# KMS-TEAM/vi_slam

Hardware: AMD Instinct MI355X
Metric: frames/sec ORB extract+match (higher is better)
Workload: dtype u8; 1 GPU; kitti00_mono_1241x376_n1000; nfeatures=1000, nlevels=8, contexts_in_flight=4, distinct_frames=32, match=SearchForInitialization(prev frame) window 100

## Files before the change

include/vslam_fe.h:

```cpp
#ifndef VSLAM_FE_H
#define VSLAM_FE_H

#include <stddef.h>
#include <stdint.h>

#ifdef __cplusplus
extern "C" {
#endif

#define VSLAM_OK 0
#define VSLAM_ERR_INVALID (-1)
#define VSLAM_ERR_NO_DEVICE (-2)
#define VSLAM_ERR_HIP (-3)
#define VSLAM_ERR_CAPACITY (-4)
#define VSLAM_ERR_UNSUPPORTED (-5)
#define VSLAM_ERR_COMM (-6)

#define VSLAM_MAX_LEVELS 16
#define VSLAM_MAX_BATCH 64

#define VSLAM_IMGS_HOST 0
#define VSLAM_IMGS_DEVICE 1
#define VSLAM_IMGS_PINNED 2
#define VSLAM_IMGS_STAGED 3

#define VSLAM_FLAG_ATAN_FMA 1u
#define VSLAM_FLAG_HOST_OCTREE 2u

typedef struct vslam_kp {
    float x, y, size, angle, response;
    int32_t octave, class_id;
} vslam_kp;

typedef struct vslam_tuning {
    int32_t pyramid_per_level;
    int32_t pyr_rows;
    int32_t pyr_threads;
    int32_t blur_rows;
    int32_t fast_threads;
    int32_t fast_pitch;
    int32_t fast_lds_pad;
    int32_t octree_walk_kernel;
    int32_t oct_fine_depth;
    int32_t oct_lds_budget_kb;
    int32_t oct_regkeys;
    int32_t oct_max_iter;
    int32_t oct_debug;
    int32_t graphs;
    int32_t h2d_route;
    int32_t d2h_route;
    int32_t copy_wgs;
    int32_t pull_depth;
    int32_t init_topm;
    int32_t init_match_host;
    int32_t sbp_topm;
    int32_t sbp_sequential;
    int32_t si_queries_per_block;
    int32_t fg_threads;
    int32_t wait_spin;
    int32_t numa;
    int32_t host_prof;
    int32_t stream_priority;
    int32_t stage_split_event;
    int32_t oct_threads;
    int32_t fast_kernel;
    int32_t fast_band_cells;
    int32_t wave_prio;
    int32_t oct_precount;
    int32_t desc_kpw;
    int32_t reserved[1];
} vslam_tuning;
void vslam_tuning_init(vslam_tuning* t);

typedef struct vslam_fe_params {
    int32_t width, height;
    int32_t nfeatures;
    float scale_factor;
    int32_t nlevels;
    int32_t ini_th_fast;
    int32_t min_th_fast;
    int32_t device;
    int32_t max_batch;
    uint32_t flags;
    int32_t gauss_taps[7];
    const vslam_tuning* tuning;
} vslam_fe_params;

typedef struct vslam_fe vslam_fe;


int vslam_fe_create(const vslam_fe_params* params, vslam_fe** out);
int vslam_fe_set_tuning(vslam_fe* fe, const vslam_tuning* t);
void vslam_fe_destroy(vslam_fe* fe);
const char* vslam_last_error(void);

int vslam_fe_tables(const vslam_fe* fe, float* scale, float* inv_scale, float* sigma2, float* inv_sigma2,
                    int32_t* features_per_level);

int vslam_fe_extract(vslam_fe* fe, const uint8_t* img, size_t pitch, int lap0, int lap1, vslam_kp* kps,
                     uint8_t* desc, int cap, int* n, int* mono_index);

int vslam_fe_extract_batch(vslam_fe* fe, int nimg, const uint8_t* const* imgs, size_t pitch,
                           int imgs_on_device, int lap0, int lap1, vslam_kp* const* kps,
                           uint8_t* const* desc, int cap, int* n, int* mono_index);

int vslam_fe_stage_images_async(vslam_fe* fe, int nimg, const uint8_t* const* imgs, size_t pitch, int imgs_where);

int vslam_fe_extract_batch_async(vslam_fe* fe, int nimg, const uint8_t* const* imgs, size_t pitch,
                                 int imgs_on_device, int lap0, int lap1, int want_host);
int vslam_fe_extract_wait(vslam_fe* fe, vslam_kp* const* kps, uint8_t* const* desc, int cap, int* n,
                          int* mono_index);

int vslam_fe_level_size(const vslam_fe* fe, int level, int* w, int* h);

int vslam_fe_capacity(const vslam_fe* fe);
int vslam_fe_level_copy(vslam_fe* fe, int slot, int level, int blurred, uint8_t* dst, size_t dst_pitch);

int vslam_fe_candidates(vslam_fe* fe, int slot, int level, vslam_kp* out, int cap);

int vslam_fe_slot_buffers(vslam_fe* fe, int slot, const vslam_kp** dev_kps, const uint8_t** dev_desc,
                          int* n);

int vslam_fe_slot_host_views(vslam_fe* fe, int slot, const vslam_kp** host_kps, const uint8_t** host_desc);

int vslam_fe_wait_for(vslam_fe* waiter, vslam_fe* signal);
int vslam_fe_event_record(vslam_fe* fe, int idx);
int vslam_fe_event_wait(vslam_fe* waiter, vslam_fe* signal, int idx);

int vslam_fe_set_fast_gate(vslam_fe* fe, vslam_fe* signal);

void* vslam_fe_stream(vslam_fe* fe);

int vslam_fe_pack_slots(vslam_fe* fe, int nslots, void* dev_dst, size_t slot_bytes);
int vslam_fe_pack_slot_range(vslam_fe* fe, int first, int nslots, void* dev_dst, size_t slot_bytes);
int vslam_fe_pack_slot_range_async(vslam_fe* fe, int first, int nslots, void* dev_dst, size_t slot_bytes);

#define VSLAM_COMM_ID_BYTES 128
typedef struct vslam_comm vslam_comm;
int vslam_comm_unique_id(uint8_t id[VSLAM_COMM_ID_BYTES]);
int vslam_comm_create(int device, int rank, int world, const uint8_t id[VSLAM_COMM_ID_BYTES], vslam_comm** out);
void vslam_comm_destroy(vslam_comm* comm);
int vslam_comm_rank(const vslam_comm* comm);
int vslam_comm_world(const vslam_comm* comm);
int vslam_exchange_ring(vslam_fe* fe, vslam_comm* comm, const void* dev_send, void* dev_recv, size_t bytes);
int vslam_exchange_allgather(vslam_fe* fe, vslam_comm* comm, const void* dev_send, void* dev_recv_all,
                             size_t bytes_per_rank);

int vslam_host_alloc(size_t bytes, void** out);
void vslam_host_free(void* p);

int vslam_fe_set_profiling(vslam_fe* fe, int on);
int vslam_fe_get_profile(vslam_fe* fe, double stage_ms[5], long* batches, long* images);
// ... 147 lines not shown

int vslam_distinctive_descriptors(vslam_fe* fe, const uint8_t* desc_host, const int32_t* offsets, int nsets,
                                  int32_t* best);

typedef struct vslam_voc vslam_voc;
int vslam_voc_create(int device, int depth_levels, int weighting, int norm, int n_nodes, const int32_t* child_start,
                     const int32_t* child_count, const int32_t* child_ids, int n_child_ids, const uint8_t* node_desc,
                     const double* node_weight, const int32_t* node_word_id, vslam_voc** out);
void vslam_voc_destroy(vslam_voc* voc);
typedef struct vslam_voc_file vslam_voc_file;
int vslam_voc_file_open(const char* path, vslam_voc_file** out);
void vslam_voc_file_close(vslam_voc_file* f);
int vslam_voc_file_info(const vslam_voc_file* f, int* branching, int* depth_levels, int* scoring, int* weighting,
                        int* norm, int* n_nodes, int* n_words, int* n_child_ids, int* format);
int vslam_voc_file_arrays(const vslam_voc_file* f, const int32_t** child_start, const int32_t** child_count,
                          const int32_t** child_ids, const uint8_t** node_desc, const double** node_weight,
                          const int32_t** node_word_id);
const char* vslam_voc_file_last_error(void);
int vslam_voc_load(int device, const char* path, vslam_voc** out);
long vslam_dbg_qlz_decode(const uint8_t* packet, size_t n, uint8_t* dst, size_t cap, size_t* used);
int vslam_voc_info(const vslam_voc* voc, int* depth_levels, int* weighting, int* norm, int* n_nodes);
int vslam_bow_transform(vslam_fe* fe, const vslam_voc* voc, const uint8_t* dev_desc, int n, int levelsup,
                        int32_t* word_id, double* weight, int32_t* node_id);
int vslam_bow_transform_slots_async(vslam_fe* fe, const vslam_voc* voc, int first_slot, int nslots, int levelsup);
int vslam_bow_transform_slots_wait(vslam_fe* fe, const int* n, int32_t* const* word_id, double* const* weight,
                                   int32_t* const* node_id);
int vslam_bow_assemble(int weighting, int norm, const int32_t* word_id, const double* weight, const int32_t* node_id,
                       int n, int32_t* bow_ids, double* bow_vals, int* n_bow, int32_t* fv_nodes, int32_t* fv_off,
                       int32_t* fv_feat, int* n_fv);

int vslam_search_by_bow(vslam_fe* fe, const vslam_kp* kf_kps_host, const uint8_t* dev_kf_desc,
                        const uint8_t* kf_flags_host, int n_kf, const int32_t* kf_fv_nodes, const int32_t* kf_fv_off,
                        const int32_t* kf_fv_feat, int n_kf_nodes, const vslam_kp* f_kps_host,
                        const uint8_t* dev_f_desc, int n_f, const int32_t* f_fv_nodes, const int32_t* f_fv_off,
                        const int32_t* f_fv_feat, int n_f_nodes, float nnratio, int check_orientation,
                        int32_t* match_f, int* nmatches);

int vslam_search_by_bow_keyframes(vslam_fe* fe, const vslam_kp* kps1_host, const uint8_t* dev_desc1,
                                  const uint8_t* flags1_host, int n1, const int32_t* fv1_nodes, const int32_t* fv1_off,
                                  const int32_t* fv1_feat, int n1_nodes, const vslam_kp* kps2_host,
                                  const uint8_t* dev_desc2, const uint8_t* flags2_host, int n2,
                                  const int32_t* fv2_nodes, const int32_t* fv2_off, const int32_t* fv2_feat,
                                  int n2_nodes, float nnratio, int check_orientation, int32_t* match12, int* nmatches);

typedef struct vslam_tri_params {
    float F12[9];
    float ep_x, ep_y;
    int32_t only_stereo, coarse, check_orientation;
} vslam_tri_params;
int vslam_search_for_triangulation(vslam_fe* fe, const vslam_tri_params* p, const vslam_kp* kps1_host,
                                   const uint8_t* dev_desc1, const uint8_t* has_mp1_host, const float* u_right1_host,
                                   int n1, const int32_t* fv1_nodes, const int32_t* fv1_off, const int32_t* fv1_feat,
                                   int n1_nodes, const vslam_kp* kps2_host, const uint8_t* dev_desc2,
                                   const uint8_t* has_mp2_host, const float* u_right2_host, int n2,
                                   const int32_t* fv2_nodes, const int32_t* fv2_off, const int32_t* fv2_feat,
                                   int n2_nodes, int32_t* match12, int* nmatches);

typedef struct vslam_fuse_point {
    float pos[3];
    float normal[3];
    float min_distance;
    float max_distance;
    int32_t valid;
} vslam_fuse_point;
typedef struct vslam_fuse_params {
    float Rcw[9], tcw[3], Ow[3];
    float fx, fy, cx, cy, bf, th;
    float log_scale_factor;
    int32_t img_w, img_h;
    int32_t sim3;
    int32_t gemm_float;
    float Rb[9], tb[3];
} vslam_fuse_params;
int vslam_fuse_search(vslam_fe* fe, const vslam_fuse_params* p, const vslam_fuse_point* points_host,
                      const uint8_t* mp_desc_host, int n_points, const vslam_kp* dev_kf_kps,
                      const uint8_t* dev_kf_desc, int n_kf, const float* kf_u_right_host, int32_t* best_idx,
                      int32_t* best_dist);

int vslam_dbg_sincos(vslam_fe* fe, const float* x, int n, float* sin_out, float* cos_out);
int vslam_dbg_fast_atan2(vslam_fe* fe, const float* y, const float* x, int n, int fma, float* deg);
int vslam_dbg_logf(vslam_fe* fe, const float* x, int n, float* y);
int vslam_fe_octree_stats(const vslam_fe* fe, unsigned long long* problems, unsigned long long* split_below_grid,
                          uint32_t* last_level_masks);
int vslam_fe_delivery_stats(const vslam_fe* fe, unsigned long long* transfers, unsigned long long* bytes);
int vslam_dbg_octree_stamps(vslam_fe* fe, unsigned long long* out64);
int vslam_dbg_search_init_fallbacks(vslam_fe* fe, int* count);
int vslam_dbg_search_init_replay_stats(vslam_fe* fe, int* rounds, int* queries, int* pairs);

#ifdef __cplusplus
}
#endif
#endif
```

vi_slam_amd/__init__.py:

```python
import ctypes as C
import os

import numpy as np

_HERE = os.path.dirname(os.path.abspath(__file__))
LIB_PATH = os.environ.get("VSLAM_FE_LIB") or os.path.join(_HERE, "libvslam_fe.so")
HOST_LIB_PATH = os.path.join(_HERE, "libvslam_host.so")

VSLAM_OK = 0
ERR_INVALID, ERR_NO_DEVICE, ERR_HIP, ERR_CAPACITY, ERR_UNSUPPORTED, ERR_COMM = -1, -2, -3, -4, -5, -6
IMGS_HOST, IMGS_DEVICE, IMGS_PINNED, IMGS_STAGED = 0, 1, 2, 3
COMM_ID_BYTES = 128
FLAG_ATAN_FMA = 1
FLAG_HOST_OCTREE = 2
MAX_BATCH = 64

KP_DTYPE = np.dtype([("x", "<f4"), ("y", "<f4"), ("size", "<f4"), ("angle", "<f4"),
                     ("response", "<f4"), ("octave", "<i4"), ("class_id", "<i4")])

ABI_SYMBOLS = [
    "vslam_fe_create", "vslam_fe_destroy", "vslam_last_error", "vslam_fe_tables", "vslam_fe_extract",
    "vslam_fe_extract_batch", "vslam_fe_level_size", "vslam_fe_level_copy", "vslam_fe_candidates",
    "vslam_fe_slot_buffers", "vslam_fe_slot_host_views", "vslam_fe_capacity", "vslam_fe_stream", "vslam_hamming_top2", "vslam_hamming_matrix",
    "vslam_stereo_match", "vslam_stereo_match_batch", "vslam_search_for_initialization",
    "vslam_dbg_sincos", "vslam_dbg_fast_atan2", "vslam_fe_pack_slots", "vslam_fe_set_profiling",
    "vslam_fe_get_profile", "vslam_fe_extract_batch_async", "vslam_fe_extract_wait",
    "vslam_search_for_initialization_batch", "vslam_frame_stereo_batch_async", "vslam_frame_stereo_wait",
    "vslam_fe_pack_slot_range", "vslam_dbg_octree_stamps", "vslam_dbg_search_init_fallbacks", "vslam_search_init_dev_async",
    "vslam_search_init_dev_wait", "vslam_fe_slot_count_ptr", "vslam_fe_pack_slot_range_async", "vslam_fe_wait_for", "vslam_fe_event_record",
    "vslam_fe_event_wait", "vslam_projection_direction", "vslam_search_by_projection_frame",
    "vslam_search_by_projection_dev_async", "vslam_search_by_projection_dev_wait", "vslam_stereo_points_dev_async",
    "vslam_stereo_points_buffers", "vslam_search_by_projection_mappoints", "vslam_distinctive_descriptors", "vslam_voc_create", "vslam_voc_destroy",
    "vslam_voc_info", "vslam_bow_transform", "vslam_bow_transform_slots_async", "vslam_bow_transform_slots_wait",
    "vslam_bow_assemble", "vslam_search_by_bow", "vslam_search_by_bow_keyframes",
    "vslam_search_for_triangulation", "vslam_fuse_search", "vslam_dbg_logf", "vslam_search_by_projection_keyframe",
    "vslam_search_by_projection_sim3",
    "vslam_comm_unique_id", "vslam_comm_create", "vslam_comm_destroy", "vslam_comm_rank", "vslam_comm_world",
    "vslam_exchange_ring", "vslam_exchange_allgather", "vslam_host_alloc", "vslam_host_free",
    "vslam_fe_stage_images_async", "vslam_fe_octree_stats", "vslam_fe_delivery_stats", "vslam_dbg_search_init_replay_stats", "vslam_tuning_init", "vslam_fe_set_tuning", "vslam_stereo_fisheye_candidates", "vslam_hamming_top2_batch", "vslam_hamming_top2_batch_dev_async", "vslam_fe_set_fast_gate",
    "vslam_voc_load", "vslam_voc_file_open", "vslam_voc_file_close", "vslam_voc_file_info", "vslam_voc_file_arrays",
    "vslam_voc_file_last_error", "vslam_dbg_qlz_decode",
    "vslam_fe_set_camera", "vslam_fe_slot_ukps", "vslam_fe_ukps_copy", "vslam_undistort_points", "vslam_fe_image_bounds",
    "vslam_fe_set_grid_bounds", "vslam_fe_get_grid_bounds",
    "vslam_search_for_initialization_ex", "vslam_search_for_initialization_batch_ex", "vslam_search_init_dev_async_ex",
]


MP_TRACK_DTYPE = np.dtype([("proj_x", "<f4"), ("proj_y", "<f4"), ("proj_xr", "<f4"), ("view_cos", "<f4"),
                           ("level", "<i4"), ("flags", "<u4")])


FUSE_POINT_DTYPE = np.dtype([("pos", "<f4", 3), ("normal", "<f4", 3), ("min_distance", "<f4"),
                             ("max_distance", "<f4"), ("valid", "<i4")])


class _TriParams(C.Structure):
    _fields_ = [("F12", C.c_float * 9), ("ep_x", C.c_float), ("ep_y", C.c_float), ("only_stereo", C.c_int32),
                ("coarse", C.c_int32), ("check_orientation", C.c_int32)]


class _FuseParams(C.Structure):
    _fields_ = [("Rcw", C.c_float * 9), ("tcw", C.c_float * 3), ("Ow", C.c_float * 3), ("fx", C.c_float),
                ("fy", C.c_float), ("cx", C.c_float), ("cy", C.c_float), ("bf", C.c_float), ("th", C.c_float),
                ("log_scale_factor", C.c_float), ("img_w", C.c_int32), ("img_h", C.c_int32), ("sim3", C.c_int32),
                ("gemm_float", C.c_int32), ("Rb", C.c_float * 9), ("tb", C.c_float * 3)]


class _ProjParams(C.Structure):
    _fields_ = [("Tcw", C.c_float * 12), ("fx", C.c_float), ("fy", C.c_float), ("cx", C.c_float), ("cy", C.c_float),
                ("mbf", C.c_float), ("th", C.c_float), ("forward", C.c_int32), ("backward", C.c_int32),
                ("check_orientation", C.c_int32), ("img_w", C.c_int32), ("img_h", C.c_int32),
                ("gemm_float", C.c_int32)]


class _SbpJob(C.Structure):
    _fields_ = [("p", _ProjParams)] + [(n, C.c_void_p) for n in (
        "dev_last_kps", "dev_n_last", "dev_last_flags", "dev_last_x3dw", "dev_mp_desc", "dev_cur_kps", "dev_cur_desc",
        "dev_n_cur", "dev_cur_u_right", "dev_cur_occupied")]


class VslamError(RuntimeError):
    def __init__(self, code, msg):
        super().__init__("vslam error %d: %s" % (code, msg))
        self.code = code


TUNING_FIELDS = ["pyramid_per_level", "pyr_rows", "pyr_threads", "blur_rows", "fast_threads", "fast_pitch", "fast_lds_pad",
                 "octree_walk_kernel", "oct_fine_depth", "oct_lds_budget_kb", "oct_regkeys", "oct_max_iter",
                 "oct_debug", "graphs", "h2d_route", "d2h_route", "copy_wgs", "pull_depth",
                 "init_topm", "init_match_host", "sbp_topm", "sbp_sequential", "si_queries_per_block", "fg_threads",
                 "wait_spin", "numa", "host_prof", "stream_priority", "stage_split_event",
                 "oct_threads", "fast_kernel", "fast_band_cells", "wave_prio", "oct_precount", "desc_kpw"]


class _Tuning(C.Structure):
    _fields_ = [(f, C.c_int32) for f in TUNING_FIELDS] + [("reserved", C.c_int32 * 1)]


def make_tuning(**kw):
    t = _Tuning()
    lib().vslam_tuning_init(C.byref(t))
    for k, v in kw.items():
        if k not in TUNING_FIELDS:
            raise KeyError("unknown tuning field %r" % k)
        setattr(t, k, int(v))
    return t


class _Params(C.Structure):
    _fields_ = [("width", C.c_int32), ("height", C.c_int32), ("nfeatures", C.c_int32),
                ("scale_factor", C.c_float), ("nlevels", C.c_int32), ("ini_th_fast", C.c_int32),
                ("min_th_fast", C.c_int32), ("device", C.c_int32), ("max_batch", C.c_int32),
                ("flags", C.c_uint32), ("gauss_taps", C.c_int32 * 7), ("tuning", C.POINTER(_Tuning))]


class _InitJob(C.Structure):
    _fields_ = [("dev_kps1", C.c_void_p), ("dev_desc1", C.c_void_p), ("dev_n1", C.c_void_p),
                ("dev_kps2", C.c_void_p), ("dev_desc2", C.c_void_p), ("dev_n2", C.c_void_p),
                ("dev_prev_matched", C.c_void_p)]


class _Camera(C.Structure):
    _fields_ = [("fx", C.c_float), ("fy", C.c_float), ("cx", C.c_float), ("cy", C.c_float), ("dist", C.c_float * 5),
                ("ndist", C.c_int32)]


class _Bounds(C.Structure):
    _fields_ = [("min_x", C.c_float), ("max_x", C.c_float), ("min_y", C.c_float), ("max_y", C.c_float)]


def _bounds(b):
    return _Bounds(*[float(v) for v in b])


def bind_voc_file(L):
    vp = C.c_void_p
    L.vslam_voc_file_open.argtypes = [C.c_char_p, vp]
    L.vslam_voc_file_close.argtypes = [vp]
    L.vslam_voc_file_close.restype = None
    L.vslam_voc_file_info.argtypes = [vp] + [vp] * 9
    L.vslam_voc_file_arrays.argtypes = [vp] + [vp] * 6
    L.vslam_voc_file_last_error.restype = C.c_char_p
    L.vslam_dbg_qlz_decode.argtypes = [C.c_char_p, C.c_size_t, vp, C.c_size_t, vp]
    L.vslam_dbg_qlz_decode.restype = C.c_long
    return L


def qlz_decode(packet, library=None, cap=None):
    L = library if library is not None else lib()
    packet = bytes(packet)
    n = len(packet)
    if cap is None:
        cap = 16 + 128 * n
    dst = C.create_string_buffer(max(cap, 1))
    used = C.c_size_t(0)
    got = L.vslam_dbg_qlz_decode(packet, n, dst, cap, C.byref(used))
    if got < 0:
        raise ValueError("damaged QuickLZ packet")
    return dst.raw[:got], used.value


_lib = None


def lib():
    global _lib
    if _lib is None:
        if not os.path.exists(LIB_PATH):
            raise ImportError("%s is missing: run `python -c 'import __graft_entry__ as g; g.build()'` "
                              "(make -C vi_slam_amd/csrc); there is no CPU fallback" % LIB_PATH)
        try:
            import torch
        except Exception:
            pass
        L = C.CDLL(LIB_PATH)
# ... 354 lines not shown
        if len(d) not in (4, 5):
            raise VslamError(ERR_INVALID, "dist must hold 4 or 5 coefficients")
        cam = _Camera(fx, fy, cx, cy, (C.c_float * 5)(*(d + [0.0] * (5 - len(d)))), len(d))
        _check(lib().vslam_fe_set_camera(self._h, C.byref(cam)))

    def slot_ukps_ptr(self, slot=0):
        k = C.c_void_p()
        _check(lib().vslam_fe_slot_ukps(self._h, slot, C.byref(k)))
        return k.value

    def ukeypoints(self, slot=0):
        out = np.zeros(self.cap, KP_DTYPE)
        n = C.c_int()
        _check(lib().vslam_fe_ukps_copy(self._h, slot, _p(out), self.cap, C.byref(n)))
        return out[:n.value].copy()

    def image_bounds(self):
        b = np.zeros(4, np.float32)
        _check(lib().vslam_fe_image_bounds(self._h, _p(b)))
        return b

    def set_grid_bounds(self, bounds):
        if bounds is None:
            _check(lib().vslam_fe_set_grid_bounds(self._h, None))
            return
        b = _bounds(bounds)
        _check(lib().vslam_fe_set_grid_bounds(self._h, C.byref(b)))

    def grid_bounds(self):
        b, s = _Bounds(), C.c_int()
        _check(lib().vslam_fe_get_grid_bounds(self._h, C.byref(b), C.byref(s)))
        return np.array([b.min_x, b.max_x, b.min_y, b.max_y], np.float32), bool(s.value)

    def wait_for(self, other):
        _check(lib().vslam_fe_wait_for(self._h, other._h))

    def event_record(self, idx):
        _check(lib().vslam_fe_event_record(self._h, idx))

    def set_fast_gate(self, other):
        L = lib()
        L.vslam_fe_set_fast_gate.argtypes = [C.c_void_p, C.c_void_p]
        _check(L.vslam_fe_set_fast_gate(self._h, other._h if other is not None else None))

    def event_wait(self, other, idx):
        _check(lib().vslam_fe_event_wait(self._h, other._h, idx))

    def stream(self):
        return lib().vslam_fe_stream(self._h)

    @property
    def slot_bytes(self):
        return (16 + self.cap * 60 + 255) & ~255

    def pack_slots(self, nslots, dev_dst, slot_bytes=None, first=0, sync=True):
        fn = lib().vslam_fe_pack_slot_range if sync else lib().vslam_fe_pack_slot_range_async
        _check(fn(self._h, first, nslots, dev_dst, slot_bytes or self.slot_bytes))

    def stereo_points_async(self, Twc, cam, observations=True, gemm_float=False):
        T = np.ascontiguousarray(np.asarray(Twc, np.float32).reshape(len(Twc), -1)[:, :12])
        _check(lib().vslam_stereo_points_dev_async(self._h, len(Twc), _p(T), C.c_float(cam[0]), C.c_float(cam[1]),
                                                   C.c_float(cam[2]), C.c_float(cam[3]), int(observations),
                                                   int(gemm_float)))

    def stereo_points_buffers(self, pair, with_stereo=True):
        x, f, u, d = C.c_void_p(), C.c_void_p(), C.c_void_p(), C.c_void_p()
        _check(lib().vslam_stereo_points_buffers(self._h, pair, C.byref(x), C.byref(f),
                                                 C.byref(u) if with_stereo else None,
                                                 C.byref(d) if with_stereo else None))
        return x.value, f.value, u.value, d.value

    def set_tuning(self, **kw):
        t = make_tuning(**kw)
        lib().vslam_fe_set_tuning.argtypes = [C.c_void_p, C.c_void_p]
        _check(lib().vslam_fe_set_tuning(self._h, C.byref(t)))

    def octree_stats(self):
        a, b = C.c_ulonglong(), C.c_ulonglong()
        m = (C.c_uint32 * MAX_BATCH)()
        lib().vslam_fe_octree_stats.argtypes = [C.c_void_p, C.c_void_p, C.c_void_p, C.c_void_p]
        _check(lib().vslam_fe_octree_stats(self._h, C.byref(a), C.byref(b), m))
        return a.value, b.value, [int(v) for v in m]

    def delivery_stats(self):
        a, b = C.c_ulonglong(), C.c_ulonglong()
        lib().vslam_fe_delivery_stats.argtypes = [C.c_void_p, C.c_void_p, C.c_void_p]
        _check(lib().vslam_fe_delivery_stats(self._h, C.byref(a), C.byref(b)))
        return a.value, b.value

    def set_profiling(self, on=True):
        _check(lib().vslam_fe_set_profiling(self._h, int(on)))

    def get_profile(self):
        ms = (C.c_double * 5)()
        b, im = C.c_long(), C.c_long()
        _check(lib().vslam_fe_get_profile(self._h, ms, C.byref(b), C.byref(im)))
        return dict(pyramid_ms=ms[0], fast_ms=ms[1], blur_ms=ms[2], describe_ms=ms[3], octree_ms=ms[4],
                    batches=b.value, images=im.value)


class FMatcher:

    TH_HIGH, TH_LOW, HISTO_LENGTH = 100, 50, 30

    def __init__(self, extractor, nnratio=0.6, checkOri=True):
        self.fe = extractor
        self.mfNNratio = nnratio
        self.mbCheckOrientation = checkOri

    def hamming_top2(self, dev_q, nq, dev_t, nt):
        idx = np.zeros((max(nq, 1), 2), np.int32)
        dist = np.zeros((max(nq, 1), 2), np.int32)
        _check(lib().vslam_hamming_top2(self.fe._h, dev_q, nq, dev_t, nt, _p(idx), _p(dist)))
        return idx[:nq], dist[:nq]

    def hamming_top2_batch(self, problems):
        n = len(problems)
        idx = [np.zeros((max(p[1], 1), 2), np.int32) for p in problems]
        dist = [np.zeros((max(p[1], 1), 2), np.int32) for p in problems]
        vp, ip = C.c_void_p * n, C.c_int32 * n
        L = lib()
        L.vslam_hamming_top2_batch.argtypes = [C.c_void_p, C.c_int, C.c_void_p, C.c_void_p, C.c_void_p, C.c_void_p, C.c_void_p, C.c_void_p]
        _check(L.vslam_hamming_top2_batch(self.fe._h, n, vp(*[p[0] for p in problems]), ip(*[p[1] for p in problems]),
                                          vp(*[p[2] for p in problems]), ip(*[p[3] for p in problems]),
                                          vp(*[a.ctypes.data for a in idx]), vp(*[a.ctypes.data for a in dist])))
        return [(idx[i][:problems[i][1]], dist[i][:problems[i][1]]) for i in range(n)]

    def hamming_top2_batch_async(self, problems):
        n = len(problems)
        vp, ip = C.c_void_p * n, C.c_int32 * n
        L = lib()
        L.vslam_hamming_top2_batch_dev_async.argtypes = [C.c_void_p, C.c_int, C.c_void_p, C.c_void_p, C.c_void_p, C.c_void_p]
        _check(L.vslam_hamming_top2_batch_dev_async(self.fe._h, n, vp(*[p[0] for p in problems]), ip(*[p[1] for p in problems]),
                                                    vp(*[p[2] for p in problems]), ip(*[p[3] for p in problems])))

    def ComputeStereoFishEyeCandidates(self, dev_desc_left, n_left, mono_left, dev_desc_right, n_right, mono_right):
        l2r = np.zeros(max(n_left, 1), np.int32)
        d0 = np.zeros(max(n_left, 1), np.int32)
        d1 = np.zeros(max(n_left, 1), np.int32)
        nc = C.c_int()
        L = lib()
        L.vslam_stereo_fisheye_candidates.argtypes = [C.c_void_p, C.c_void_p, C.c_int, C.c_int, C.c_void_p, C.c_int, C.c_int,
                                                      C.c_void_p, C.c_void_p, C.c_void_p, C.c_void_p]
        _check(L.vslam_stereo_fisheye_candidates(self.fe._h, dev_desc_left, n_left, mono_left, dev_desc_right, n_right,
                                                 mono_right, _p(l2r), _p(d0), _p(d1), C.byref(nc)))
        return l2r[:n_left], d0[:n_left], d1[:n_left], nc.value

    def hamming_matrix(self, dev_q, nq, dev_t, nt):
        out = np.zeros((max(nq, 1), max(nt, 1)), np.uint8)
        _check(lib().vslam_hamming_matrix(self.fe._h, dev_q, nq, dev_t, nt, _p(out)))
        return out[:nq, :nt]

    def SearchForInitialization(self, kps1, dev_desc1, kps2, dev_desc2, vbPrevMatched, windowSize=10,
                                img_size=None, bounds=None):
        kps1 = np.ascontiguousarray(kps1, KP_DTYPE)
        kps2 = np.ascontiguousarray(kps2, KP_DTYPE)
        pm = np.ascontiguousarray(vbPrevMatched, np.float32).copy()
        m = np.full(max(len(kps1), 1), -1, np.int32)
        nm = C.c_int(0)
        if bounds is not None:
            _check(lib().vslam_search_for_initialization_ex(self.fe._h, _p(kps1), dev_desc1, len(kps1), _p(kps2),
                                                            dev_desc2, len(kps2), C.byref(_bounds(bounds)), _p(pm), _p(m),
                                                            windowSize, self.mfNNratio, int(self.mbCheckOrientation),
                                                            C.byref(nm)))
            return nm.value, m[:len(kps1)], pm
        w, h = img_size or (self.fe.width, self.fe.height)
# ... 484 lines not shown
```

vi_slam_amd/csrc/vslam_ctx.h:

```cpp
#ifndef VSLAM_CTX_H
#define VSLAM_CTX_H
#include <hip/hip_runtime.h>

#include <algorithm>
#include <atomic>
#include <cmath>
#include <condition_variable>
#include <cstdio>
#include <cstring>
#include <functional>
#include <mutex>
#include <string>
#include <thread>
#include <vector>

#include "../../include/vslam_orb_pattern.h"
#include "vslam_host.h"
#include "vslam_pool.h"
#include "vslam_kernels.h"
#include "vslam_tuning.h"

std::string& vslam_err();
#define g_err (vslam_err())

#define HIPCHK(call)                                                                             \
    do {                                                                                         \
        hipError_t e_ = (call);                                                                  \
        if (e_ != hipSuccess) {                                                                  \
            g_err = std::string(#call) + ": " + hipGetErrorString(e_);                           \
            return VSLAM_ERR_HIP;                                                                \
        }                                                                                        \
    } while (0)

enum { VSLAM_REGION_NONE = 0, VSLAM_REGION_INIT = 1, VSLAM_REGION_STEREO = 2 };
struct vslam_fe {
    vslam_fe_params p;
    vslam_tuning tune;
    vslam::ExtractorTables tab;
    PyramidGeom geom;
    size_t slot_stride = 0;
    int B = 1, cap = 0;

    hipStream_t stream = nullptr;
    hipEvent_t ev_cand = nullptr;
    hipEvent_t ev_x = nullptr;
    hipEvent_t ev_user[4] = {};
    int desc_kpw_hint = -1;
    hipEvent_t ev_fast = nullptr;
    vslam_fe* fast_gate = nullptr;
    bool fast_gated_by_someone = false;
    std::vector<vslam_fe*> gate_waiters;

    uint8_t* d_pyr = nullptr;
    uint8_t* d_blur = nullptr;
    uint16_t* d_xtab[VSLAM_MAX_LEVELS] = {};
    int16_t* d_xa[VSLAM_MAX_LEVELS] = {};
    uint16_t* d_ytab[VSLAM_MAX_LEVELS] = {};
    int16_t* d_yb[VSLAM_MAX_LEVELS] = {};
    uint16_t* d_qbase[VSLAM_MAX_LEVELS] = {};
    ResizeQuad* d_quads[VSLAM_MAX_LEVELS] = {};
    struct PyrGroupCtx {
        PyrGroupDev dev;
        size_t lds_bytes;
        PyrTileDev* d_tiles;
    };
    std::vector<PyrGroupCtx> pyr_groups;
    std::vector<vslam::HostCell> cells;
    int level_cell_first[VSLAM_MAX_LEVELS + 1] = {};
    CellDesc* d_cells = nullptr;
    int tile_pitch = 0, tile_rows = 0, max_px = 0;
    BandDesc* d_bands = nullptr;
    uint8_t* d_band_classes = nullptr;
    int nbands = 0, band_max_wh = 0, band_max_iw = 0;
    uint8_t* d_cand = nullptr;
    uint8_t* h_cand = nullptr;
    size_t cand_stride = 0;
    int cand_cap = 0;
    int32_t taps[7];
    uint32_t* d_blur_tasks = nullptr;
    int n_blur_tasks = 0;
    int oct_threads = 1024;
    int blur_rows = 32;
    SelKp* d_sel = nullptr;
    SelKp* h_sel = nullptr;
    uint8_t* d_res = nullptr;
    uint8_t* h_res = nullptr;
    size_t res_bytes = 0, res_counts_bytes = 0, res_feat_bytes = 0, res_init_bytes = 0;
    bool init_in_block = false;
    unsigned long long n_deliveries = 0, n_delivery_bytes = 0, graph_deliveries = 0, graph_delivery_bytes = 0;
    bool deliver_deferred = false;
    vslam_kp* d_kps = nullptr;
    uint8_t* d_desc = nullptr;
    vslam_kp* h_kps = nullptr;
    uint8_t* h_desc = nullptr;
    int8_t* d_pattern = nullptr;
    BatchSrc src;
    int n_out[VSLAM_MAX_BATCH] = {};
    int mono_out[VSLAM_MAX_BATCH] = {};
    unsigned long long oct_problems = 0, oct_deep = 0;
    uint32_t oct_last_mask[VSLAM_MAX_BATCH] = {};
    int32_t pack_hdr[VSLAM_MAX_BATCH][4] = {};
    std::vector<std::vector<vslam::Cand>> sel_level;
    std::vector<std::vector<vslam::Cand>> cand_level;
    uint8_t* h_top2 = nullptr;
    size_t h_top2_bytes = 0;
    uint32_t* d_part = nullptr;
    size_t part_bytes = 0;
    int32_t* d_idx2 = nullptr;
    int32_t* d_dist2 = nullptr;
    size_t top2_cap = 0;
    uint8_t* d_dmat = nullptr;
    size_t dmat_bytes = 0;
    uint8_t* d_tmp_desc[2] = {nullptr, nullptr};
    size_t tmp_desc_bytes[2] = {0, 0};
    uint8_t* d_init = nullptr;
    size_t init_bytes = 0;
    uint8_t* h_init = nullptr;
    size_t h_init_bytes = 0;
    int init_pairs = 0;
    bool init_lds_set = false;
    bool has_cam = false;
    UdCam ud;
    vslam_kp* d_ukps = nullptr;
    bool has_grid_bounds = false;
    SiBounds grid_bounds = {0.0f, 0.0f, 0.0f, 0.0f};
    uint8_t* d_init_scratch = nullptr;
    size_t init_scratch_bytes = 0;
    int* d_init_fb = nullptr;
    uint8_t* d_proj = nullptr;
    size_t proj_bytes = 0;
    uint8_t* h_proj = nullptr;
    size_t h_proj_bytes = 0;
    bool proj_lds_set = false, dist_lds_set = false;
    uint8_t* d_bow = nullptr;
    size_t bow_bytes = 0;
    uint8_t* h_bow = nullptr;
    size_t h_bow_bytes = 0;
    int bow_jobs = 0;
    bool use_graph = true;
    hipGraphExec_t graph_exec = nullptr;
    long long graph_key = 0;
    size_t graph_pitch = 0;
    const uint8_t* graph_imgs[VSLAM_MAX_BATCH] = {};
    int graph_lap0 = 0, graph_lap1 = 0;
    uint8_t* h_img = nullptr;
    size_t h_img_pitch = 0;
    uint8_t* d_stage = nullptr;
    size_t d_stage_bytes = 0;
    uint8_t* d_sbp = nullptr;
// ... 81 lines not shown
```

vi_slam_amd/csrc/vslam_fe.hip:

```cpp
#if defined(__SSE2__)
#include <emmintrin.h>
#endif
#include "vslam_ctx.h"

#include <algorithm>
#include <chrono>
#include <mutex>
#include <cstdio>
#include <cstdlib>

void vslam_host_prof_report();

std::string& vslam_err() {
    static thread_local std::string e;
    return e;
}
extern "C" const char* vslam_last_error(void) { return vslam_err().c_str(); }

static std::mutex g_gate_mu;

static void gate_unlink(vslam_fe* fe) {
    if (fe->fast_gate) {
        auto& w = fe->fast_gate->gate_waiters;
        w.erase(std::remove(w.begin(), w.end(), fe), w.end());
// ... 74 lines not shown
        if (fe->ev_prof[i]) hipEventDestroy(fe->ev_prof[i]);
    if (fe->stream) hipStreamDestroy(fe->stream);
    delete fe;
}

extern "C" void vslam_fe_destroy(vslam_fe* fe) {
    if (fe) hipSetDevice(fe->p.device);
    vslam_host_prof_report();
    free_ctx(fe);
}

#define UPLOAD(dst, ptr, bytes)                                                                  \
    do {                                                                                         \
        const size_t n_ = (bytes);                                                               \
        HIPCHK(hipMalloc((void**)&(dst), n_ ? n_ : 4));                                          \
        if (n_) HIPCHK(hipMemcpy((dst), (ptr), n_, hipMemcpyHostToDevice));                      \
    } while (0)


static int create_geometry(vslam_fe* fe) {
    const vslam_fe_params& p = fe->p;
    vslam::build_tables(p.nfeatures, p.scale_factor, p.nlevels, fe->tab);
    fe->B = p.max_batch;
    static const int32_t def_taps[7] = {18, 34, 48, 56, 48, 34, 18};
    bool zero = true;
    for (int i = 0; i < 7; i++) zero = zero && p.gauss_taps[i] == 0;
    for (int i = 0; i < 7; i++) fe->taps[i] = zero ? def_taps[i] : p.gauss_taps[i];

    memset(&fe->geom, 0, sizeof(fe->geom));
    fe->geom.nlevels = p.nlevels;
    int lws[VSLAM_MAX_LEVELS], lhs[VSLAM_MAX_LEVELS];
    size_t off = 0;
    for (int l = 0; l < p.nlevels; l++) {
        int lw, lh;
        vslam::level_size(fe->tab, p.width, p.height, l, &lw, &lh);
        LevelGeom& g = fe->geom.lv[l];
        g.w = lws[l] = lw;
        g.h = lhs[l] = lh;
        g.pitch = (lw + 127) & ~127;
        g.off = (uint32_t)off;
        g.scale = fe->tab.scale[l];
        off += (size_t)g.pitch * lh;
        off = (off + 255) & ~(size_t)255;
        if (lw < 40 || lh < 40 || lw > 4095 + 32 || lh > 4095 + 32) {
            g_err = "image too small/large for this level count";
            return VSLAM_ERR_UNSUPPORTED;
        }
        if ((int)std::round((float)(lw - 32) / (float)(lh - 32)) < 1) {
            g_err = "portrait aspect ratio: the reference's DistributeOctTree has nIni == 0 (undefined)";
            return VSLAM_ERR_UNSUPPORTED;
        }
    }
    fe->slot_stride = off;
    fe->cap = vslam::keypoint_capacity(fe->tab.quota.data(), lws, lhs, p.nlevels, p.nfeatures);
    HIPCHK(hipMalloc((void**)&fe->d_pyr, fe->slot_stride * fe->B));
    HIPCHK(hipMalloc((void**)&fe->d_blur, fe->slot_stride * fe->B));
    HIPCHK(hipMemset(fe->d_pyr, 0, fe->slot_stride * fe->B));
    HIPCHK(hipMemset(fe->d_blur, 0, fe->slot_stride * fe->B));
    return VSLAM_OK;
}

static int create_pyramid(vslam_fe* fe) {
    const vslam_fe_params& p = fe->p;
    std::vector<vslam::PyrLevelTables> pyr_tabs(p.nlevels);
    for (int l = 1; l < p.nlevels; l++) {
        vslam::ResizeTables& r = pyr_tabs[l].r;
        const LevelGeom &s = fe->geom.lv[l - 1], &d = fe->geom.lv[l];
        pyr_tabs[l].sw = s.w; pyr_tabs[l].sh = s.h; pyr_tabs[l].dw = d.w; pyr_tabs[l].dh = d.h;
        vslam::build_resize_tables(s.w, s.h, d.w, d.h, r);
        UPLOAD(fe->d_xtab[l], r.xtab.data(), r.xtab.size() * 2);
        UPLOAD(fe->d_xa[l], r.xa.data(), r.xa.size() * 2);
        UPLOAD(fe->d_ytab[l], r.ytab.data(), r.ytab.size() * 2);
        UPLOAD(fe->d_yb[l], r.yb.data(), r.yb.size() * 2);
        std::vector<uint16_t>& qbase = pyr_tabs[l].qbase;
        std::vector<uint32_t>& quads = pyr_tabs[l].quads;
        if (vslam::build_resize_quads(r, s.w, d.w, qbase, quads)) {
            UPLOAD(fe->d_qbase[l], qbase.data(), qbase.size() * 2);
            UPLOAD(fe->d_quads[l], quads.data(), quads.size() * 4);
        } else {
            qbase.clear();
            quads.clear();
        }
    }
    bool fused = fe->tune.pyramid_per_level != 1 && p.nlevels > 1;
    for (int l = 1; l < p.nlevels && fused; l++) fused = fe->d_quads[l] != nullptr;
    static_assert(sizeof(PyrTileDev) == sizeof(vslam::PyrTileLevel), "planner and kernel share the tile record");
    const int pyr_rows = fe->tune.pyr_rows >= 0 ? fe->tune.pyr_rows
                         : fe->B <= 2 ? 16 : (size_t)p.width * p.height > 1000000 ? 40 : 48;
#ifndef VSLAM_PYR_LDS_KB
#define VSLAM_PYR_LDS_KB 64
#endif
    for (int l0 = 0; fused && l0 + 1 < p.nlevels;) {
        const int nl = std::min(l0 == 0 ? 3 : VSLAM_PYR_GROUP_LEVELS, p.nlevels - 1 - l0);
        std::vector<const vslam::PyrLevelTables*> gt;
        for (int j = 1; j <= nl; j++) gt.push_back(&pyr_tabs[l0 + j]);
        vslam::PyrGroupPlan plan;
        if (!vslam::build_pyramid_group(gt, l0, VSLAM_PYR_LDS_KB * 1024, plan, pyr_rows)) {
            fused = false;
            break;
        }
        vslam_fe::PyrGroupCtx g;
        memset(&g.dev, 0, sizeof(g.dev));
        g.dev.l0 = l0;
        g.dev.nl = nl;
        g.dev.ntiles = plan.ntx * plan.nty;
        g.dev.readable_w0 = p.width;
        g.lds_bytes = plan.lds_bytes;
        g.d_tiles = nullptr;
        UPLOAD(g.d_tiles, plan.tiles.data(), plan.tiles.size() * sizeof(PyrTileDev));
        g.dev.tiles = g.d_tiles;
        for (int j = 0; j <= nl; j++) g.dev.lg[j] = fe->geom.lv[l0 + j];
        for (int j = 1; j <= nl; j++) {
            g.dev.qbase[j - 1] = fe->d_qbase[l0 + j];
            g.dev.quads[j - 1] = fe->d_quads[l0 + j];
            g.dev.ytab[j - 1] = fe->d_ytab[l0 + j];
            g.dev.yb[j - 1] = fe->d_yb[l0 + j];
        }
        fe->pyr_groups.push_back(g);
        l0 += nl;
    }
    if (!fused) {
        for (auto& g : fe->pyr_groups) hipFree(g.d_tiles);
        fe->pyr_groups.clear();
    }
    return VSLAM_OK;
}

static int create_fast(vslam_fe* fe) {
    const vslam_fe_params& p = fe->p;
    for (int l = 0; l < p.nlevels; l++) {
        fe->level_cell_first[l] = (int)fe->cells.size();
        vslam::build_cells(l, fe->geom.lv[l].w, fe->geom.lv[l].h, fe->cells);
    }
    fe->level_cell_first[p.nlevels] = (int)fe->cells.size();
    if (fe->cells.empty()) {
        g_err = "image too small: no 30-px FAST cell fits on any pyramid level";
        return VSLAM_ERR_UNSUPPORTED;
    }
    int maxw = 8, maxh = 8;
    size_t cand_total = 0;
    std::vector<CellDesc> dc(fe->cells.size());
    for (size_t i = 0; i < fe->cells.size(); i++) {
        const vslam::HostCell& c = fe->cells[i];
        dc[i].level = c.level; dc[i].x0 = c.x0; dc[i].y0 = c.y0; dc[i].x1 = c.x1; dc[i].y1 = c.y1; dc[i].pad = 0;
        dc[i].base = (uint32_t)cand_total;
        cand_total += (size_t)((c.x1 - c.x0 - 6 + 1) / 2) * (size_t)((c.y1 - c.y0 - 6 + 1) / 2);
        maxw = std::max(maxw, c.x1 - c.x0);
        maxh = std::max(maxh, c.y1 - c.y0);
    }
    fe->tile_pitch = (maxw + 3) & ~3;
    fe->tile_rows = maxh;
    fe->max_px = (maxw - 6) * (maxh - 6);
    if (fe->max_px > 8192) {
        g_err = "FAST cell larger than 8192 px";
        return VSLAM_ERR_UNSUPPORTED;
    }
    if (maxw > 66 || maxh > 134 || fe->geom.lv[p.nlevels - 1].w < 8) {
        g_err = "FAST cell window larger than 66 x 134 px";
        return VSLAM_ERR_UNSUPPORTED;
    }
    UPLOAD(fe->d_cells, dc.data(), dc.size() * sizeof(CellDesc));
    std::vector<vslam::HostBand> hb;
    vslam::build_bands(fe->cells, std::min(4, std::max(1, tune_or(fe->tune.fast_band_cells, 4))), 128, hb);
    vslam::BandTables bt;
    vslam::pack_bands(hb, p.nlevels, bt);
    static_assert(sizeof(BandDesc) == sizeof(vslam::BandWords), "packer and kernel share the band record");
    if (bt.ok && vk_fast_bands_check(bt.max_wh, bt.max_iw, bt.max_cells) == 0) {
        UPLOAD(fe->d_band_classes, bt.classes.data(), bt.classes.size());
        UPLOAD(fe->d_bands, bt.bands.data(), bt.bands.size() * sizeof(BandDesc));
        fe->nbands = (int)bt.bands.size();
        fe->band_max_wh = bt.max_wh;
        fe->band_max_iw = bt.max_iw;
    }
    fe->cand_cap = (int)std::max<size_t>(cand_total, 16);
    fe->cand_stride = (8 + fe->cells.size() * sizeof(CellOut) + (size_t)fe->cand_cap * 4 + 255) & ~(size_t)255;
    HIPCHK(hipMalloc((void**)&fe->d_cand, fe->cand_stride * fe->B));
    HIPCHK((hipError_t)vslam_pinned_alloc((void**)&fe->h_cand, fe->cand_stride * fe->B));
    return VSLAM_OK;
}

static int create_blur(vslam_fe* fe) {
    UPLOAD(fe->d_pattern, VSLAM_ORB_PATTERN, 1024);
    vk_upload_disc(fe->tab.umax);
    if (fe->tune.blur_rows >= 0) fe->blur_rows = std::min(512, std::max(8, (int)fe->tune.blur_rows));
    else if (fe->B <= 2) fe->blur_rows = 8;
    std::vector<uint32_t> tasks;
    for (int l = 0; l < fe->p.nlevels; l++) {
        const int br = fe->blur_rows;
        const int ns = std::max(1, (fe->geom.lv[l].w + 247) / 248), nc = (fe->geom.lv[l].h + br - 1) / br;
        for (int c = 0; c < nc; c++)
            for (int s = 0; s < ns; s++) tasks.push_back(((uint32_t)l << 24) | ((uint32_t)c << 12) | (uint32_t)s);
    }
    fe->n_blur_tasks = (int)tasks.size();
    UPLOAD(fe->d_blur_tasks, tasks.data(), tasks.size() * 4);
    return VSLAM_OK;
}

static int create_result_block(vslam_fe* fe) {
    const size_t nk = (size_t)fe->B * fe->cap;
    HIPCHK(hipMalloc((void**)&fe->d_sel, nk * sizeof(SelKp)));
    HIPCHK((hipError_t)vslam_pinned_alloc((void**)&fe->h_sel, nk * sizeof(SelKp)));
    fe->res_counts_bytes = (((size_t)(fe->B * 4 + 4) * 4) + 255) & ~(size_t)255;
    fe->res_feat_bytes = fe->res_counts_bytes + nk * sizeof(vslam_kp) + nk * 32;
    fe->res_init_bytes = (nk * 12 + (size_t)fe->B * 16 + 255) & ~(size_t)255;
    fe->res_bytes = fe->res_feat_bytes + fe->res_init_bytes;
    HIPCHK(hipMalloc((void**)&fe->d_res, fe->res_bytes));
    HIPCHK((hipError_t)vslam_pinned_alloc((void**)&fe->h_res, fe->res_bytes));
    HIPCHK(hipMemset(fe->d_res, 0, fe->res_bytes));
    memset(fe->h_res, 0, fe->res_bytes);
    fe->d_counts = (int32_t*)fe->d_res;
    fe->h_counts = (int32_t*)fe->h_res;
    fe->d_kps = (vslam_kp*)(fe->d_res + fe->res_counts_bytes);
    fe->h_kps = (vslam_kp*)(fe->h_res + fe->res_counts_bytes);
    fe->d_desc = fe->d_res + fe->res_counts_bytes + nk * sizeof(vslam_kp);
    fe->h_desc = fe->h_res + fe->res_counts_bytes + nk * sizeof(vslam_kp);
    fe->d_init = fe->d_res + fe->res_feat_bytes;
    fe->h_init = fe->h_res + fe->res_feat_bytes;
    fe->init_bytes = fe->h_init_bytes = fe->res_init_bytes;
    fe->init_in_block = true;
    return VSLAM_OK;
}

static int create_quadtree(vslam_fe* fe) {
    const vslam_fe_params& p = fe->p;
    int lws[VSLAM_MAX_LEVELS], lhs[VSLAM_MAX_LEVELS];
    for (int l = 0; l < p.nlevels; l++) {
        lws[l] = fe->geom.lv[l].w;
        lhs[l] = fe->geom.lv[l].h;
    }
    const size_t budget = (size_t)std::min(150, std::max(16, tune_or(fe->tune.oct_lds_budget_kb, 128))) * 1024;
    vslam::OctPlan plan;
    vslam::plan_octree(fe->tab.quota.data(), lws, lhs, fe->level_cell_first, p.nlevels, fe->tune.oct_fine_depth, budget,
                       vk_octree_lds_bytes, plan);
    OctParams& O = fe->oct;
    memset(&O, 0, sizeof(O));
    for (int l = 0; l < p.nlevels; l++) {
        O.N[l] = plan.N[l]; O.H[l] = plan.H[l]; O.nIni[l] = plan.nIni[l]; O.hX[l] = plan.hX[l];
        O.selOff[l] = plan.selOff[l]; O.fineD[l] = plan.fineD[l]; O.lutOff[l] = plan.lutOff[l]; O.lutW[l] = plan.lutW[l];
    }
    for (int l = 0; l <= p.nlevels; l++) O.cellFirst[l] = fe->level_cell_first[l];
    O.selStride = plan.selStride;
    O.maxNodes = plan.maxNodes;
    O.fineLdsOff = plan.fineLdsOff;
    O.fineLdsBytes = plan.fineLdsBytes;
    O.ptsCap = fe->cand_cap;
    if (fe->tune.oct_debug == 1) {
        HIPCHK(hipMalloc(&O.dbg, 64 * 8));
        HIPCHK(hipMemset(O.dbg, 0, 64 * 8));
    }
    O.maxIter = tune_or(fe->tune.oct_max_iter, 64);
    const bool on_device = fe->dev_octree = plan.fits && !(p.flags & VSLAM_FLAG_HOST_OCTREE);
    fe->oct_threads = fe->tune.oct_threads == 256 || fe->tune.oct_threads == 512 || fe->tune.oct_threads == 1024
                          ? fe->tune.oct_threads
                          : fe->B <= 2 ? 1024 : (size_t)p.width * p.height > 1000000 ? 512 : 256;
    if (!on_device) return VSLAM_OK;
    if (vk_octree_set_max_lds((size_t)O.fineLdsOff + (size_t)O.fineLdsBytes + 16) != 0) {
        g_err = "hipFuncSetAttribute(k_octree, max dynamic LDS) failed";
        return VSLAM_ERR_HIP;
    }
    const size_t np = (size_t)fe->B * fe->cand_cap;
    HIPCHK(hipMalloc((void**)&fe->d_pts[0], np * 4));
    HIPCHK(hipMalloc((void**)&fe->d_pts[1], np * 4));
    HIPCHK(hipMalloc((void**)&fe->d_sel_xyr, (size_t)fe->B * O.selStride * 4));
    HIPCHK(hipMalloc((void**)&fe->d_sel_cnt, (size_t)fe->B * VSLAM_MAX_LEVELS * 4));
    HIPCHK(hipMalloc((void**)&fe->d_oct_sorted, np * 8));
    HIPCHK(hipMalloc((void**)&fe->d_oct_redo, (size_t)fe->B * VSLAM_MAX_LEVELS * 4));
    HIPCHK(hipMemset(fe->d_oct_redo, 0, (size_t)fe->B * VSLAM_MAX_LEVELS * 4));
    UPLOAD(fe->d_oct_lut, plan.lut.data(), plan.lut.size() * 4);
    O.lut = fe->d_oct_lut;
    return VSLAM_OK;
}

static int create_stream_and_pool(vslam_fe* fe) {
    const int pr = tune_or(fe->tune.stream_priority, 0);
    int lo = 0, hi = 0;
    if (pr != 0 && hipDeviceGetStreamPriorityRange(&lo, &hi) == hipSuccess && lo != hi)
        HIPCHK(hipStreamCreateWithPriority(&fe->stream, hipStreamNonBlocking, pr == 1 ? lo : hi));
// ... 8 lines not shown
    nthreads = std::min(nthreads, fe->B * fe->p.nlevels - 1);
    fe->pool = new WorkerPool(std::max(nthreads, 0));
    return VSLAM_OK;
}

static int create_impl(vslam_fe* fe) {
    int ndev = 0;
    if (hipGetDeviceCount(&ndev) != hipSuccess || ndev <= 0 || fe->p.device >= ndev) {
        g_err = "no usable HIP device (this library has no CPU fallback)";
        return VSLAM_ERR_NO_DEVICE;
    }
    HIPCHK(hipSetDevice(fe->p.device));
    int (*const steps[])(vslam_fe*) = {create_geometry, create_pyramid, create_fast, create_blur, create_result_block,
                                       create_quadtree, create_stream_and_pool};
    for (auto step : steps) {
        const int rc = step(fe);
        if (rc != VSLAM_OK) return rc;
    }
    HIPCHK(hipDeviceSynchronize());
    return VSLAM_OK;
}

extern "C" int vslam_fe_create(const vslam_fe_params* p, vslam_fe** out) {
    if (!p || !out) return VSLAM_ERR_INVALID;
    *out = nullptr;
    if (p->width <= 0 || p->height <= 0 || p->nfeatures <= 0 || p->nlevels < 1 ||
        p->nlevels > VSLAM_MAX_LEVELS || p->scale_factor <= 1.0f || p->max_batch < 1 ||
        p->max_batch > VSLAM_MAX_BATCH || p->min_th_fast < 1 || p->ini_th_fast < p->min_th_fast ||
        p->ini_th_fast > 254 || p->nfeatures > 60000) {
        g_err = "invalid parameters";
        return VSLAM_ERR_INVALID;
    }
    vslam_fe* fe = new vslam_fe();
    fe->p = *p;
    fe->tune = vslam_resolve_tuning(p->tuning);
    fe->p.tuning = nullptr;
    int rc = create_impl(fe);
    if (rc != VSLAM_OK) {
        std::string keep = g_err;
        free_ctx(fe);
        g_err = keep;
        return rc;
    }
    *out = fe;
    return VSLAM_OK;
}

extern "C" int vslam_fe_set_tuning(vslam_fe* fe, const vslam_tuning* t) {
    if (!fe || !t) return VSLAM_ERR_INVALID;
    vslam_apply_tuning(fe->tune, t);
    fe->use_graph = fe->use_graph && fe->tune.graphs != 0;
    if (fe->graph_exec) {
        if (fe->stream) hipStreamSynchronize(fe->stream);
        hipGraphExecDestroy(fe->graph_exec);
        fe->graph_exec = nullptr;
        fe->graph_key = 0;
    }
    return VSLAM_OK;
}

extern "C" int vslam_fe_tables(const vslam_fe* fe, float* scale, float* inv_scale, float* sigma2,
                               float* inv_sigma2, int32_t* quota) {
    if (!fe) return VSLAM_ERR_INVALID;
    for (int i = 0; i < fe->p.nlevels; i++) {
        if (scale) scale[i] = fe->tab.scale[i];
        if (inv_scale) inv_scale[i] = fe->tab.inv_scale[i];
        if (sigma2) sigma2[i] = fe->tab.sigma2[i];
        if (inv_sigma2) inv_sigma2[i] = fe->tab.inv_sigma2[i];
        if (quota) quota[i] = fe->tab.quota[i];
    }
    return fe->p.nlevels;
}

extern "C" int vslam_fe_octree_stats(const vslam_fe* fe, unsigned long long* problems, unsigned long long* split_below_grid,
                                     uint32_t* last_level_masks) {
    if (!fe) return VSLAM_ERR_INVALID;
    if (problems) *problems = fe->oct_problems;
    if (split_below_grid) *split_below_grid = fe->oct_deep;
    if (last_level_masks)
        for (int s = 0; s < fe->B; s++) last_level_masks[s] = s < fe->last_nimg ? fe->oct_last_mask[s] : 0u;
    return VSLAM_OK;
}

extern "C" int vslam_fe_delivery_stats(const vslam_fe* fe, unsigned long long* transfers, unsigned long long* bytes) {
    if (!fe) return VSLAM_ERR_INVALID;
    if (transfers) *transfers = fe->n_deliveries;
    if (bytes) *bytes = fe->n_delivery_bytes;
    return VSLAM_OK;
}

extern "C" int vslam_dbg_octree_stamps(vslam_fe* fe, unsigned long long* out64) {
    if (!fe || !fe->oct.dbg) return VSLAM_ERR_INVALID;
    HIPCHK(hipMemcpy(out64, fe->oct.dbg, 64 * 8, hipMemcpyDeviceToHost));
    return VSLAM_OK;
}

extern "C" void* vslam_fe_stream(vslam_fe* fe) { return fe ? (void*)fe->stream : nullptr; }

extern "C" int vslam_fe_wait_for(vslam_fe* waiter, vslam_fe* signal) {
    if (!waiter || !signal || waiter->p.device != signal->p.device) return VSLAM_ERR_INVALID;
    if (waiter == signal) return VSLAM_OK;
    HIPCHK(hipSetDevice(waiter->p.device));
    if (!signal->ev_x) HIPCHK(hipEventCreateWithFlags(&signal->ev_x, hipEventDisableTiming));
    HIPCHK(hipEventRecord(signal->ev_x, signal->stream));
    HIPCHK(hipStreamWaitEvent(waiter->stream, signal->ev_x, 0));
    return VSLAM_OK;
}

extern "C" int vslam_fe_event_record(vslam_fe* fe, int idx) {
    if (!fe || idx < 0 || idx >= 4) return VSLAM_ERR_INVALID;
    HIPCHK(hipSetDevice(fe->p.device));
    if (!fe->ev_user[idx]) HIPCHK(hipEventCreateWithFlags(&fe->ev_user[idx], hipEventDisableTiming));
    HIPCHK(hipEventRecord(fe->ev_user[idx], fe->stream));
    return VSLAM_OK;
}

extern "C" int vslam_fe_event_wait(vslam_fe* waiter, vslam_fe* signal, int idx) {
    if (!waiter || !signal || idx < 0 || idx >= 4 || waiter->p.device != signal->p.device) return VSLAM_ERR_INVALID;
    if (!signal->ev_user[idx] || waiter == signal) return VSLAM_OK;
    HIPCHK(hipSetDevice(waiter->p.device));
    HIPCHK(hipStreamWaitEvent(waiter->stream, signal->ev_user[idx], 0));
    return VSLAM_OK;
}

extern "C" int vslam_fe_set_fast_gate(vslam_fe* fe, vslam_fe* signal) {
    if (!fe || (signal && (signal == fe || signal->p.device != fe->p.device))) return VSLAM_ERR_INVALID;
    std::lock_guard<std::mutex> lk(g_gate_mu);
    gate_unlink(fe);
    if (signal) {
        fe->fast_gate = signal;
        signal->gate_waiters.push_back(fe);
        HIPCHK(hipSetDevice(signal->p.device));
        if (!signal->ev_fast) HIPCHK(hipEventCreateWithFlags(&signal->ev_fast, hipEventDisableTiming));
        signal->fast_gated_by_someone = true;
        fe->use_graph = false;
        signal->use_graph = false;
    }
    return VSLAM_OK;
}

extern "C" int vslam_fe_set_profiling(vslam_fe* fe, int on) {
    if (!fe) return VSLAM_ERR_INVALID;
    HIPCHK(hipSetDevice(fe->p.device));
    if (on && !fe->ev_prof[0])
        for (int i = 0; i < 10; i++) HIPCHK(hipEventCreate(&fe->ev_prof[i]));
    fe->profiling = on != 0;
    for (int i = 0; i < 5; i++) fe->prof_ms[i] = 0;
    fe->prof_batches = fe->prof_images = 0;
    return VSLAM_OK;
}

extern "C" int vslam_fe_get_profile(vslam_fe* fe, double stage_ms[5], long* batches, long* images) {
    if (!fe || !stage_ms) return VSLAM_ERR_INVALID;
    for (int i = 0; i < 5; i++) stage_ms[i] = fe->prof_ms[i];
    if (batches) *batches = fe->prof_batches;
    if (images) *images = fe->prof_images;
    return VSLAM_OK;
}

static int pack_range(vslam_fe* fe, int first, int nslots, void* dev_dst, size_t slot_bytes, bool sync) {
    if (!fe || first < 0 || nslots < 0 || first + nslots > fe->B || !dev_dst ||
        slot_bytes < 16 + (size_t)fe->cap * 60 || (slot_bytes & 15) || ((uintptr_t)dev_dst & 15)) {
        g_err = "invalid arguments (slot_bytes and dev_dst must be 16-byte aligned)";
        return VSLAM_ERR_INVALID;
    }
    HIPCHK(hipSetDevice(fe->p.device));
// ... 128 lines not shown
    const bool use_sdma = h2d_uses_sdma(fe, nimg);
    BatchSrc hs;
    for (int s = 0; s < nimg; s++) {
        if (where == VSLAM_IMGS_PINNED && !imgs[s]) {
            g_err = "null image";
            return VSLAM_ERR_INVALID;
        }
        hs.l0[s] = where == VSLAM_IMGS_PINNED ? imgs[s] : fe->h_img + img_bytes * s;
        hs.pitch0[s] = where == VSLAM_IMGS_PINNED ? (uint32_t)pitch : (uint32_t)fe->h_img_pitch;
    }
    int from_host = 1;
    if (use_sdma) {
        const size_t spitch = hs.pitch0[0];
        const size_t one = (size_t)(p.height - 1) * spitch + p.width;
        const size_t stride = (one + 255) & ~(size_t)255;
        if (fe->d_stage_bytes < stride * fe->B + 256) {
            g_err = "internal: device staging buffer not allocated";
            return VSLAM_ERR_HIP;
        }
        hipStream_t cs = st;
        bool even = nimg > 1;
        const ptrdiff_t d = nimg > 1 ? hs.l0[1] - hs.l0[0] : 0;
        for (int s = 2; s < nimg && even; s++) even = hs.l0[s] - hs.l0[s - 1] == d;
        if (even && d > 0 && (size_t)d >= one && (size_t)d * (nimg - 1) + one <= fe->d_stage_bytes) {
            const int ek = fe->tune.stage_split_event;
            const int h1 = nimg / 2;
            if (ek >= 0 && ek < 4 && h1 >= 1 && !hip_stream_capturing(cs)) {
                HIPCHK(hipMemcpyAsync(fe->d_stage, hs.l0[0], (size_t)d * h1, hipMemcpyHostToDevice, cs));
                if (!fe->ev_user[ek]) HIPCHK(hipEventCreateWithFlags(&fe->ev_user[ek], hipEventDisableTiming));
                HIPCHK(hipEventRecord(fe->ev_user[ek], cs));
                HIPCHK(hipMemcpyAsync(fe->d_stage + (size_t)d * h1, hs.l0[0] + (size_t)d * h1, (size_t)d * (nimg - 1 - h1) + one,
                                      hipMemcpyHostToDevice, cs));
            } else
                HIPCHK(hipMemcpyAsync(fe->d_stage, hs.l0[0], (size_t)d * (nimg - 1) + one, hipMemcpyHostToDevice, cs));
            for (int s = 0; s < nimg; s++) hs.l0[s] = fe->d_stage + (size_t)d * s;
        } else {
            for (int s = 0; s < nimg; s++) {
                HIPCHK(hipMemcpyAsync(fe->d_stage + stride * s, hs.l0[s], one, hipMemcpyHostToDevice, cs));
                hs.l0[s] = fe->d_stage + stride * s;
            }
        }
        from_host = 0;
    }
    vk_pull_images(st, hs, fe->d_pyr, fe->slot_stride, fe->geom.lv[0].off, (int)lp, p.width, p.height, nimg, from_host, fe->tune);
    return VSLAM_OK;
}

static void src_at_slots(vslam_fe* fe, int nimg) {
    for (int s = 0; s < nimg; s++) {
        fe->src.l0[s] = fe->d_pyr + (size_t)s * fe->slot_stride + fe->geom.lv[0].off;
        fe->src.pitch0[s] = (uint32_t)fe->geom.lv[0].pitch;
    }
}

static int enqueue_front(vslam_fe* fe, int nimg, const uint8_t* const* imgs, size_t pitch, int on_device) {
    const vslam_fe_params& p = fe->p;
    const int L = p.nlevels;
    hipStream_t st = fe->stream;
    if (on_device == VSLAM_IMGS_DEVICE) {
        for (int s = 0; s < nimg; s++) {
            if (!imgs[s]) {
                g_err = "null image";
                return VSLAM_ERR_INVALID;
            }
            fe->src.l0[s] = imgs[s];
            fe->src.pitch0[s] = (uint32_t)pitch;
        }
    } else {
        if (on_device != VSLAM_IMGS_STAGED) {
            int rc = upload_host_rows(fe, nimg, imgs, pitch, on_device);
            if (rc) return rc;
        }
        src_at_slots(fe, nimg);
    }
    fe->last_nimg = nimg;
    fe->cand_on_host = false;
    int32_t* d_errw = fe->dev_octree ? fe->d_counts + (size_t)fe->B * 4 : nullptr;
    if (fe->pyr_groups.empty()) vk_reset_headers(st, fe->d_cand, fe->cand_stride, nimg, d_errw);
    const bool prof = fe->profiling;
    if (prof) HIPCHK(hipEventRecord(fe->ev_prof[0], st));
    bool first_group = true;
    for (const auto& g : fe->pyr_groups) {
        vk_pyramid_group(st, fe->d_pyr, fe->slot_stride, fe->src, g.dev, g.lds_bytes, nimg,
                         first_group ? fe->d_cand : nullptr, fe->cand_stride, first_group ? d_errw : nullptr);
        first_group = false;
    }
    for (int l = 1; l < L && fe->pyr_groups.empty(); l++) {
        if (fe->d_quads[l])
            vk_resize_level_v2(st, fe->d_pyr, fe->slot_stride, fe->src, fe->geom.lv[l - 1], fe->geom.lv[l], l - 1,
                               fe->d_qbase[l], fe->d_quads[l], fe->d_ytab[l], fe->d_yb[l], nimg);
        else
            vk_resize_level(st, fe->d_pyr, fe->slot_stride, fe->src, fe->geom.lv[l - 1], fe->geom.lv[l], l - 1,
                            fe->d_xtab[l], fe->d_xa[l], fe->d_ytab[l], fe->d_yb[l], nimg);
    }
    if (prof) HIPCHK(hipEventRecord(fe->ev_prof[1], st));
    if (fe->fast_gate && fe->fast_gate->ev_fast) HIPCHK(hipStreamWaitEvent(st, fe->fast_gate->ev_fast, 0));
    if (fe->nbands > 0 && tune_or(fe->tune.fast_kernel, fe->B <= 2 ? 3 : 4) != 3)
        vk_fast_bands(st, fe->d_pyr, fe->slot_stride, fe->src, fe->geom, fe->d_bands, fe->nbands, fe->d_band_classes, fe->d_cells,
                      (int)fe->cells.size(), fe->d_cand, fe->cand_stride, p.ini_th_fast, p.min_th_fast, fe->band_max_wh, fe->band_max_iw, nimg);
    else
        vk_fast_cells_v3(st, fe->d_pyr, fe->slot_stride, fe->src, fe->geom, fe->d_cells, (int)fe->cells.size(), fe->d_cand,
                         fe->cand_stride, p.ini_th_fast, p.min_th_fast, fe->tile_rows, fe->tile_pitch, fe->max_px, nimg);
    if (fe->fast_gated_by_someone && fe->ev_fast) HIPCHK(hipEventRecord(fe->ev_fast, st));
    if (prof) HIPCHK(hipEventRecord(fe->ev_prof[2], st));
    return VSLAM_OK;
}

static int fetch_candidates(vslam_fe* fe, int nimg) {
    const size_t hdr_bytes = 8 + fe->cells.size() * sizeof(CellOut);
    HIPCHK(hipMemcpy2DAsync(fe->h_cand, fe->cand_stride, fe->d_cand, fe->cand_stride, hdr_bytes + (size_t)fe->cand_cap * 4,
                            nimg, hipMemcpyDeviceToHost, fe->stream));
    HIPCHK(hipEventRecord(fe->ev_cand, fe->stream));
    return VSLAM_OK;
}

static int wait_candidates(vslam_fe* fe, int nimg) {
    HIPCHK(hipEventSynchronize(fe->ev_cand));
    for (int s = 0; s < nimg; s++) {
        const uint32_t* hdr = (const uint32_t*)(fe->h_cand + (size_t)s * fe->cand_stride);
        if (hdr[1]) {
            g_err = "FAST candidate buffer overflow";
            return VSLAM_ERR_CAPACITY;
        }
    }
    fe->cand_on_host = true;
    return VSLAM_OK;
}

static int enqueue_blur(vslam_fe* fe, int nimg) {
    if (fe->profiling) HIPCHK(hipEventRecord(fe->ev_prof[3], fe->stream));
    vk_blur7_v2(fe->stream, fe->d_pyr, fe->slot_stride, fe->src, fe->geom, fe->d_blur, fe->d_blur_tasks,
                fe->n_blur_tasks, fe->taps, fe->blur_rows, nimg);
    if (fe->profiling) HIPCHK(hipEventRecord(fe->ev_prof[4], fe->stream));
    return VSLAM_OK;
}

static int select_host(vslam_fe* fe, int nimg, int lap0, int lap1) {
    const int L = fe->p.nlevels;
    hipStream_t st = fe->stream;
    int rc = fetch_candidates(fe, nimg);
    if (rc == VSLAM_OK) rc = enqueue_blur(fe, nimg);
    if (rc) return rc;
    HIPCHK(hipGetLastError());
    if ((rc = wait_candidates(fe, nimg))) return rc;
    std::atomic<int> bad(0);
    fe->pool->parallel_for(nimg * L, [&](int task) {
        const int s = task / L, l = task % L;
        decode_candidates(fe, s, l);
        const std::vector<vslam::Cand>& cl = fe->cand_level[(size_t)s * L + l];
        const LevelGeom& g = fe->geom.lv[l];
        if (!vslam::distribute_octree(cl.data(), (int)cl.size(), g.w - 2 * VSLAM_FAST_BORDER,
                                      g.h - 2 * VSLAM_FAST_BORDER, fe->tab.quota[l],
                                      fe->sel_level[(size_t)s * L + l]))
            bad++;
    });
    if (bad.load()) {
        g_err = "DistributeOctTree: nIni == 0";
        return VSLAM_ERR_UNSUPPORTED;
    }
    for (int s = 0; s < nimg; s++) {
        int nk = 0;
        for (int l = 0; l < L; l++) nk += (int)fe->sel_level[(size_t)s * L + l].size();
        if (nk > fe->cap) {
            g_err = "internal keypoint capacity exceeded";
            return VSLAM_ERR_CAPACITY;
        }
        SelKp* sel = fe->h_sel + (size_t)s * fe->cap;
        int monoIndex = 0, stereoIndex = nk - 1;
        for (int l = 0; l < L; l++) {
            const float scale = fe->tab.scale[l];
            for (const vslam::Cand& c : fe->sel_level[(size_t)s * L + l]) {
                const int lx = c.x + VSLAM_FAST_BORDER, ly = c.y + VSLAM_FAST_BORDER;
                float px = (float)lx;
                if (l != 0) px = px * scale;
                SelKp k;
                k.x = (uint16_t)lx;
                k.y = (uint16_t)ly;
                k.level = (uint8_t)l;
                k.slot = (uint8_t)s;
                k.response = c.response;
                k.pad = 0;
                k.out = (px >= (float)lap0 && px <= (float)lap1) ? (uint32_t)stereoIndex-- : (uint32_t)monoIndex++;
                *sel++ = k;
            }
        }
        fe->h_counts[s * 4] = nk;
        fe->h_counts[s * 4 + 1] = monoIndex;
        fe->h_counts[s * 4 + 2] = 0;
    }
    fe->h_counts[fe->B * 4] = 0;
    HIPCHK(hipMemcpyAsync(fe->d_counts, fe->h_counts, (size_t)(fe->B * 4 + 4) * 4, hipMemcpyHostToDevice, st));
    HIPCHK(hipMemcpyAsync(fe->d_sel, fe->h_sel, (size_t)nimg * fe->cap * sizeof(SelKp), hipMemcpyHostToDevice, st));
    if (fe->profiling) {
        HIPCHK(hipEventRecord(fe->ev_prof[7], st));
        HIPCHK(hipEventRecord(fe->ev_prof[8], st));
    }
    return VSLAM_OK;
}

static int select_dev(vslam_fe* fe, int nimg, int lap0, int lap1) {
    hipStream_t st = fe->stream;
    int32_t* d_err = fe->d_counts + (size_t)fe->B * 4;
    const int rc = enqueue_blur(fe, nimg);
    if (rc) return rc;
    if (fe->profiling) HIPCHK(hipEventRecord(fe->ev_prof[7], st));
    vk_octree(st, fe->d_cand, fe->cand_stride, (int)fe->cells.size(), fe->oct, fe->d_pts[0], fe->d_pts[1],
              fe->d_oct_sorted, (size_t)fe->cand_cap, fe->d_sel_xyr, fe->d_sel_cnt, d_err, fe->p.nlevels, nimg,
              fe->d_oct_redo, fe->tune.oct_regkeys, fe->oct_threads);
    vk_assign_out(st, fe->oct, fe->geom, fe->d_sel_xyr, fe->d_sel_cnt, lap0, lap1, fe->d_sel, fe->d_counts, fe->cap,
                  d_err, nimg, fe->d_oct_redo);
    if (fe->profiling) HIPCHK(hipEventRecord(fe->ev_prof[8], st));
    return VSLAM_OK;
}

static int enqueue_back(vslam_fe* fe, int nimg, int lap0, int lap1) {
// ... 582 lines not shown
```

vi_slam_amd/csrc/vslam_host.cpp:

```cpp
#include "vslam_host.h"
#include "vslam_undistort.h"

#include <algorithm>
#include <climits>
#include <cmath>
#include <cstdlib>
#include <cstring>

namespace vslam {

static inline int cv_round(float v) { return (int)lrintf(v); }
static inline int cv_round(double v) { return (int)lrint(v); }
static inline int cv_floor(float v) {
    int i = (int)v;
    return i - (i > v);
}
static inline int cv_ceil(float v) {
    int i = (int)v;
    return i + (i < v);
}
static inline int16_t sat_short(float v) {
    int iv = cv_round(v);
    return (int16_t)std::min(std::max(iv, (int)SHRT_MIN), (int)SHRT_MAX);
}
// ... 32 lines not shown
    for (v = 0; v <= vmax; ++v) t.umax[v] = cv_round(sqrt(hp2 - v * v));
    for (v = HP, v0 = 0; v >= vmin; --v) {
        while (t.umax[v0] == t.umax[v0 + 1]) ++v0;
        t.umax[v] = v0;
        ++v0;
    }
    t.disc_u.clear();
    t.disc_v.clear();
    for (v = -HP; v <= HP; v++) {
        const int d = t.umax[std::abs(v)];
        for (int u = -d; u <= d; u++) {
            t.disc_u.push_back((int8_t)u);
            t.disc_v.push_back((int8_t)v);
        }
    }
}

void level_size(const ExtractorTables& t, int w, int h, int level, int* lw, int* lh) {
    const float scale = t.inv_scale[level];
    *lw = cv_round((float)w * scale);
    *lh = cv_round((float)h * scale);
}

void build_resize_tables(int sw, int sh, int dw, int dh, ResizeTables& r) {
    const int ONE = 2048;
    const double scale_x = 1. / ((double)dw / sw), scale_y = 1. / ((double)dh / sh);
    r.xtab.resize(2 * dw);
    r.xa.resize(2 * dw);
    r.ytab.resize(2 * dh);
    r.yb.resize(2 * dh);
    for (int dx = 0; dx < dw; dx++) {
        float fx = (float)((dx + 0.5) * scale_x - 0.5);
        int sx = cv_floor(fx);
        fx -= sx;
        if (sx < 0) { fx = 0; sx = 0; }
        if (sx >= sw - 1) { fx = 0; sx = sw - 1; }
        r.xtab[2 * dx] = (uint16_t)sx;
        r.xtab[2 * dx + 1] = (uint16_t)std::min(sx + 1, sw - 1);
        r.xa[2 * dx] = sat_short((1.f - fx) * ONE);
        r.xa[2 * dx + 1] = sat_short(fx * ONE);
    }
    auto clip = [](int x, int a, int b) { return x >= a ? (x < b ? x : b - 1) : a; };
    for (int dy = 0; dy < dh; dy++) {
        float fy = (float)((dy + 0.5) * scale_y - 0.5);
        int sy = cv_floor(fy);
        fy -= sy;
        r.ytab[2 * dy] = (uint16_t)clip(sy, 0, sh);
        r.ytab[2 * dy + 1] = (uint16_t)clip(sy + 1, 0, sh);
        r.yb[2 * dy] = sat_short((1.f - fy) * ONE);
        r.yb[2 * dy + 1] = sat_short(fy * ONE);
    }
}

bool build_resize_quads(const ResizeTables& r, int sw, int dw, std::vector<uint16_t>& qbase,
                        std::vector<uint32_t>& quads) {
    if (sw < 8) return false;
    const int nq = (dw + 3) / 4;
    qbase.assign(nq, 0);
    quads.assign((size_t)nq * 8, 0);
    for (int q = 0; q < nq; q++) {
        int lo = 1 << 30, hi = -1;
        for (int j = 0; j < 4; j++) {
            const int dx = std::min(4 * q + j, dw - 1);
            lo = std::min(lo, (int)r.xtab[2 * dx]);
            hi = std::max(hi, (int)r.xtab[2 * dx + 1]);
        }
        const int base = std::min(lo, sw - 8);
        if (hi - base > 7) return false;
        qbase[q] = (uint16_t)base;
        for (int j = 0; j < 4; j++) {
            const int dx = std::min(4 * q + j, dw - 1);
            const uint32_t o0 = r.xtab[2 * dx] - base, o1 = r.xtab[2 * dx + 1] - base;
            quads[(size_t)q * 8 + j] = o0 | (0x0cu << 8) | (o1 << 16) | (0x0cu << 24);
            quads[(size_t)q * 8 + 4 + j] = (uint32_t)(uint16_t)r.xa[2 * dx] | ((uint32_t)(uint16_t)r.xa[2 * dx + 1] << 16);
        }
    }
    return true;
}


static inline int div_floor4(int x) { return x >> 2; }

static bool plan_with(const std::vector<const PyrLevelTables*>& tabs, int l0, int ntx, int nty, size_t max_lds,
                      PyrGroupPlan& plan) {
    const int nl = (int)tabs.size();
    plan.l0 = l0;
    plan.nl = nl;
    plan.ntx = ntx;
    plan.nty = nty;
    plan.tiles.assign((size_t)ntx * nty * (nl + 1), PyrTileLevel{});
    size_t lds_max = 0;
    for (int ty = 0; ty < nty; ty++)
        for (int tx = 0; tx < ntx; tx++) {
            PyrTileLevel* T = &plan.tiles[((size_t)ty * ntx + tx) * (nl + 1)];
            int cq0[VSLAM_MAX_LEVELS + 1], cq1[VSLAM_MAX_LEVELS + 1], cr0[VSLAM_MAX_LEVELS + 1], cr1[VSLAM_MAX_LEVELS + 1];
            int nq0 = -1, nq1 = -1, nr0 = -1, nr1 = -1;
            for (int j = nl; j >= 0; j--) {
                int oq0 = 0, oq1 = 0, or0 = 0, or1 = 0;
                if (j >= 1) {
                    const PyrLevelTables& t = *tabs[j - 1];
                    const int nq = (t.dw + 3) / 4;
                    oq0 = (int)((long long)tx * nq / ntx);
                    oq1 = (int)((long long)(tx + 1) * nq / ntx);
                    or0 = (int)((long long)ty * t.dh / nty);
                    or1 = (int)((long long)(ty + 1) * t.dh / nty);
                    T[j].sq0 = (int16_t)oq0; T[j].sq1 = (int16_t)oq1; T[j].sr0 = (int16_t)or0; T[j].sr1 = (int16_t)or1;
                }
                const bool own = j >= 1 && oq1 > oq0 && or1 > or0, need = nq1 > nq0 && nr1 > nr0;
                if (!own && !need) { cq0[j] = cq1[j] = cr0[j] = cr1[j] = 0; }
                else if (own && need) {
                    cq0[j] = std::min(oq0, nq0); cq1[j] = std::max(oq1, nq1);
                    cr0[j] = std::min(or0, nr0); cr1[j] = std::max(or1, nr1);
                } else if (own) { cq0[j] = oq0; cq1[j] = oq1; cr0[j] = or0; cr1[j] = or1; }
                else { cq0[j] = nq0; cq1[j] = nq1; cr0[j] = nr0; cr1[j] = nr1; }
                nq0 = nq1 = nr0 = nr1 = -1;
                if (j >= 1 && cq1[j] > cq0[j]) {
                    const PyrLevelTables& t = *tabs[j - 1];
                    const int dxl = std::min(4 * cq1[j], t.dw) - 1;
                    const int lo = t.qbase[cq0[j]];
                    const int hi = t.r.xtab[2 * dxl + 1];
                    nq0 = div_floor4(lo);
                    nq1 = div_floor4(hi) + 1;
                    nr0 = t.r.ytab[2 * cr0[j]];
                    nr1 = t.r.ytab[2 * (cr1[j] - 1) + 1] + 1;
                }
            }
            size_t off = 0;
            for (int j = 0; j <= nl; j++) {
                T[j].c0 = (int16_t)(4 * cq0[j]);
                T[j].nc = (int16_t)(4 * (cq1[j] - cq0[j]));
                T[j].r0 = (int16_t)cr0[j];
                T[j].nr = (int16_t)(cr1[j] - cr0[j]);
                T[j].pitch = (uint32_t)((T[j].nc + 8 + 15) & ~15);
                T[j].lds_off = (uint32_t)off;
                off += (size_t)T[j].pitch * T[j].nr;
                if (j >= 1 && T[j].nc / 4 > 64) return false;
                if (j == 0 && T[j].pitch / 16 > 64) return false;
            }
            for (int j = 1; j <= nl; j++) {
                T[j].rt_off = (uint32_t)off;
                off += ((size_t)T[j].nr * 8 + 15) & ~(size_t)15;
            }
            lds_max = std::max(lds_max, off + 16);
        }
    plan.lds_bytes = lds_max;
    return lds_max <= max_lds;
}

bool build_pyramid_group(const std::vector<const PyrLevelTables*>& tabs, int l0, size_t max_lds, PyrGroupPlan& plan, int rows_override) {
    if (tabs.empty() || tabs.size() > VSLAM_MAX_LEVELS) return false;
    for (const PyrLevelTables* t : tabs)
        if (!t || t->qbase.empty()) return false;
    const int nq1 = (tabs[0]->dw + 3) / 4, h1 = tabs[0]->dh;
    int rows = 48;
    if (rows_override >= 0) rows = std::min(64, std::max(4, rows_override));
    const int nty = std::max(1, (h1 + rows - 1) / rows);
#ifndef VSLAM_PYR_TILE_QUADS
#define VSLAM_PYR_TILE_QUADS 52
#endif
    for (int ntx = std::max(1, (nq1 + VSLAM_PYR_TILE_QUADS - 1) / VSLAM_PYR_TILE_QUADS); ntx <= std::max(1, nq1 / 8); ntx++)
        if (plan_with(tabs, l0, ntx, nty, max_lds, plan)) return true;
    return false;
}

int emulate_pyramid_group(const PyrGroupPlan& plan, const std::vector<const PyrLevelTables*>& tabs,
                          const uint8_t* src, int sstride, int readable_w, std::vector<uint8_t*>& dst,
                          const std::vector<int>& dstride) {
    const int nl = plan.nl;
    std::vector<uint8_t> lds(plan.lds_bytes), ok(plan.lds_bytes);
    for (int tile = 0; tile < plan.ntx * plan.nty; tile++) {
        const PyrTileLevel* T = &plan.tiles[(size_t)tile * (nl + 1)];
        std::fill(lds.begin(), lds.end(), (uint8_t)0xCD);
        std::fill(ok.begin(), ok.end(), (uint8_t)0);
        if (T[0].nr <= 0 || T[0].nc <= 0) continue;
        for (int r = 0; r < T[0].nr; r++)
            for (int c = 0; c < (int)T[0].pitch; c++) {
                const int col = T[0].c0 + c;
                const size_t a = T[0].lds_off + (size_t)r * T[0].pitch + c;
                if (a >= lds.size()) return -1;
                if (col < readable_w) {
                    lds[a] = src[(size_t)(T[0].r0 + r) * sstride + col];
                    ok[a] = 1;
                }
            }
        for (int j = 1; j <= nl; j++) {
            const PyrLevelTables& t = *tabs[j - 1];
            const PyrTileLevel &S = T[j - 1], &D = T[j];
            for (int r = D.r0; r < D.r0 + D.nr; r++) {
                const int sy0 = t.r.ytab[2 * r], sy1 = t.r.ytab[2 * r + 1], b0 = t.r.yb[2 * r], b1 = t.r.yb[2 * r + 1];
                if (sy0 < S.r0 || sy1 >= S.r0 + S.nr) return -2;
                for (int lane = 0; lane < D.nc / 4; lane++) {
                    const int q = D.c0 / 4 + lane;
                    const int loc = (int)t.qbase[q] - S.c0;
                    if (loc < 0) return -3;
                    const int dwb = loc & ~3, sh = loc & 3;
                    if (dwb + 12 > (int)S.pitch) return -4;
                    uint32_t out = 0;
                    for (int k = 0; k < 4; k++) {
                        const uint32_t sel = t.quads[(size_t)q * 8 + k], cf = t.quads[(size_t)q * 8 + 4 + k];
                        const int o0 = sel & 0xFF, o1 = (sel >> 16) & 0xFF;
                        const int a0 = (int16_t)(cf & 0xFFFF), a1 = (int16_t)(cf >> 16);
                        int h[2];
                        for (int rr = 0; rr < 2; rr++) {
                            const size_t base = S.lds_off + (size_t)((rr ? sy1 : sy0) - S.r0) * S.pitch + dwb + sh;
                            if (base + 8 > lds.size()) return -5;
                            if (!ok[base + o0] || !ok[base + o1]) return -6;
                            h[rr] = lds[base + o0] * a0 + lds[base + o1] * a1;
                        }
                        const int v = (((b0 * (h[0] >> 4)) >> 16) + ((b1 * (h[1] >> 4)) >> 16) + 2) >> 2;
                        out |= (uint32_t)(v & 0xFF) << (8 * k);
                    }
                    const size_t da = D.lds_off + (size_t)(r - D.r0) * D.pitch + 4 * lane;
                    if (da + 4 > lds.size()) return -7;
                    for (int k = 0; k < 4; k++) {
                        lds[da + k] = (uint8_t)(out >> (8 * k));
                        ok[da + k] = 1;
                    }
                    if (q >= D.sq0 && q < D.sq1 && r >= D.sr0 && r < D.sr1)
                        for (int k = 0; k < 4; k++)
                            if (4 * q + k < dstride[j]) dst[j][(size_t)r * dstride[j] + 4 * q + k] = (uint8_t)(out >> (8 * k));
                }
            }
        }
    }
    return 0;
}

void build_cells(int level, int lw, int lh, std::vector<HostCell>& out) {
    const float W = 30;
    const int minBorderX = VSLAM_FAST_BORDER, minBorderY = VSLAM_FAST_BORDER;
    const int maxBorderX = lw - VSLAM_FAST_BORDER, maxBorderY = lh - VSLAM_FAST_BORDER;
    const float width = (float)(maxBorderX - minBorderX);
    const float height = (float)(maxBorderY - minBorderY);
    const int nCols = (int)(width / W);
    const int nRows = (int)(height / W);
    if (nCols < 1 || nRows < 1) return;
    const int wCell = (int)std::ceil(width / nCols);
    const int hCell = (int)std::ceil(height / nRows);
    for (int i = 0; i < nRows; i++) {
        const float iniY = (float)(minBorderY + i * hCell);
        float maxY = iniY + hCell + 6;
        if (iniY >= maxBorderY - 3) continue;
        if (maxY > maxBorderY) maxY = (float)maxBorderY;
        for (int j = 0; j < nCols; j++) {
            const float iniX = (float)(minBorderX + j * wCell);
            float maxX = iniX + wCell + 6;
            if (iniX >= maxBorderX - 6) continue;
            if (maxX > maxBorderX) maxX = (float)maxBorderX;
            HostCell c;
            c.level = (uint16_t)level;
            c.x0 = (uint16_t)iniX;
            c.y0 = (uint16_t)iniY;
            c.x1 = (uint16_t)maxX;
            c.y1 = (uint16_t)maxY;
            if (c.x1 - c.x0 < 7 || c.y1 - c.y0 < 7) continue;
            out.push_back(c);
        }
    }
}

void build_bands(const std::vector<HostCell>& cells, int max_cells, int max_width, std::vector<HostBand>& out) {
    const size_t n = cells.size();
    size_t i = 0;
    while (i < n) {
        size_t e = i + 1;
        while (e < n && cells[e].level == cells[i].level && cells[e].y0 == cells[i].y0 && cells[e].y1 == cells[i].y1 &&
               cells[e].x0 > cells[e - 1].x0)
            e++;
        const int nrow = (int)(e - i);
        const int wcell = nrow > 1 ? cells[i + 1].x0 - cells[i].x0 : std::max(1, cells[i].x1 - cells[i].x0 - 6);
        const int per = std::max(1, std::min(max_cells, max_width / std::max(wcell, 1)));
        for (size_t b = i; b < e; b += (size_t)per) {
            const size_t last = std::min(e, b + (size_t)per) - 1;
            HostBand hb;
            hb.cell0 = (uint32_t)b;
            hb.level = cells[b].level;
            hb.ncell = (uint16_t)(last - b + 1);
            hb.wcell = (uint16_t)wcell;
            hb.x0 = cells[b].x0;
            hb.y0 = cells[b].y0;
            hb.ww = (uint16_t)(cells[last].x1 - cells[b].x0);
            hb.wh = (uint16_t)(cells[b].y1 - cells[b].y0);
            out.push_back(hb);
        }
        i = e;
    }
}

namespace {
struct QNode {
    int x0, y0, x1, y1;
    int begin, count;
    int prev, next;
    bool noMore;
};

struct QTree {
    std::vector<QNode> pool;
    std::vector<int> perm, tmp;
    const Cand* c;
    int head = -1, tail = -1, size = 0;

    int push_front(const QNode& n) {
        int id = (int)pool.size();
        pool.push_back(n);
// ... 400 lines not shown
        }
        if (bestDist <= TH_LOW) {
            if (bestDist < (float)bestDist2 * mfNNratio) {
                if (vnMatches21[bestIdx2] >= 0) {
                    vnMatches12[vnMatches21[bestIdx2]] = -1;
                    nmatches--;
                }
                vnMatches12[i1] = bestIdx2;
                vnMatches21[bestIdx2] = i1;
                vMatchedDistance[bestIdx2] = bestDist;
                nmatches++;
                if (checkOri) {
                    float rot = kps1[i1].angle - kps2[bestIdx2].angle;
                    if (rot < 0.0) rot += 360.0f;
                    int bin = (int)std::round(rot * factor);
                    if (bin == HISTO_LENGTH) bin = 0;
                    rotHist[bin].push_back(i1);
                }
            }
        }
    }
    if (checkOri) {
        int ind1 = -1, ind2 = -1, ind3 = -1;
        int sizes[30];
        for (int i = 0; i < HISTO_LENGTH; i++) sizes[i] = (int)rotHist[i].size();
        compute_three_maxima(sizes, HISTO_LENGTH, ind1, ind2, ind3);
        for (int i = 0; i < HISTO_LENGTH; i++) {
            if (i == ind1 || i == ind2 || i == ind3) continue;
            for (int idx1 : rotHist[i])
                if (vnMatches12[idx1] >= 0) {
                    vnMatches12[idx1] = -1;
                    nmatches--;
                }
        }
    }
    for (int i1 = 0; i1 < n1; i1++)
        if (vnMatches12[i1] >= 0) {
            prevMatched[2 * i1] = kps2[vnMatches12[i1]].x;
            prevMatched[2 * i1 + 1] = kps2[vnMatches12[i1]].y;
        }
    return nmatches;
}

}

extern "C" {

int vslamh_tables(int nfeatures, float scale, int nlevels, float* sf, float* isf, float* s2, float* is2,
                  int* quota, int* umax16, int* disc_n) {
    vslam::ExtractorTables t;
    vslam::build_tables(nfeatures, scale, nlevels, t);
    for (int i = 0; i < nlevels; i++) {
        sf[i] = t.scale[i]; isf[i] = t.inv_scale[i]; s2[i] = t.sigma2[i]; is2[i] = t.inv_sigma2[i];
        quota[i] = t.quota[i];
    }
    for (int i = 0; i < 16; i++) umax16[i] = t.umax[i];
    *disc_n = (int)t.disc_u.size();
    return 0;
}

int vslamh_level_size(int nfeatures, float scale, int nlevels, int w, int h, int level, int* lw, int* lh) {
    vslam::ExtractorTables t;
    vslam::build_tables(nfeatures, scale, nlevels, t);
    vslam::level_size(t, w, h, level, lw, lh);
    return 0;
}

int vslamh_resize_with_tables(const uint8_t* src, int sw, int sh, size_t sstride, uint8_t* dst, int dw, int dh,
                              size_t dstride) {
    vslam::ResizeTables r;
    vslam::build_resize_tables(sw, sh, dw, dh, r);
    for (int dy = 0; dy < dh; dy++)
        for (int dx = 0; dx < dw; dx++) {
            const uint8_t* r0 = src + (size_t)r.ytab[2 * dy] * sstride;
            const uint8_t* r1 = src + (size_t)r.ytab[2 * dy + 1] * sstride;
            const int sx0 = r.xtab[2 * dx], sx1 = r.xtab[2 * dx + 1], a0 = r.xa[2 * dx], a1 = r.xa[2 * dx + 1];
            const int h0 = r0[sx0] * a0 + r0[sx1] * a1, h1 = r1[sx0] * a0 + r1[sx1] * a1;
            const int b0 = r.yb[2 * dy], b1 = r.yb[2 * dy + 1];
            dst[(size_t)dy * dstride + dx] = (uint8_t)((((b0 * (h0 >> 4)) >> 16) + ((b1 * (h1 >> 4)) >> 16) + 2) >> 2);
        }
    return 0;
}

int vslamh_pyramid_fused(const uint8_t* img, int w, int h, size_t stride, int nfeatures, float scale, int nlevels,
                         uint8_t* out, int* lds_bytes_max, int* tiles_total) {
    vslam::ExtractorTables t;
    vslam::build_tables(nfeatures, scale, nlevels, t);
    std::vector<vslam::PyrLevelTables> tabs(nlevels);
    std::vector<int> lw(nlevels), lh(nlevels);
    for (int l = 0; l < nlevels; l++) vslam::level_size(t, w, h, l, &lw[l], &lh[l]);
    for (int l = 1; l < nlevels; l++) {
        vslam::PyrLevelTables& T = tabs[l];
        T.sw = lw[l - 1]; T.sh = lh[l - 1]; T.dw = lw[l]; T.dh = lh[l];
        vslam::build_resize_tables(T.sw, T.sh, T.dw, T.dh, T.r);
        if (!vslam::build_resize_quads(T.r, T.sw, T.dw, T.qbase, T.quads)) return -100;
    }
    std::vector<std::vector<uint8_t>> lv(nlevels);
    std::vector<int> pitch(nlevels);
    for (int l = 0; l < nlevels; l++) {
        pitch[l] = (lw[l] + 127) & ~127;
        lv[l].assign((size_t)pitch[l] * lh[l], 0xEE);
    }
    for (int y = 0; y < h; y++) memcpy(&lv[0][(size_t)y * pitch[0]], img + (size_t)y * stride, w);
    int ngroups = 0;
    *lds_bytes_max = 0;
    *tiles_total = 0;
    for (int l0 = 0; l0 + 1 < nlevels;) {
        const int nl = std::min(l0 == 0 ? 3 : 4, nlevels - 1 - l0);
        std::vector<const vslam::PyrLevelTables*> gt;
        for (int j = 1; j <= nl; j++) gt.push_back(&tabs[l0 + j]);
        vslam::PyrGroupPlan plan;
        if (!vslam::build_pyramid_group(gt, l0, 64 * 1024, plan)) return -101;
        std::vector<uint8_t*> dst(nl + 1, nullptr);
        std::vector<int> ds(nl + 1, 0);
        for (int j = 1; j <= nl; j++) { dst[j] = lv[l0 + j].data(); ds[j] = pitch[l0 + j]; }
        const int rc = vslam::emulate_pyramid_group(plan, gt, lv[l0].data(), pitch[l0], l0 == 0 ? w : pitch[l0], dst, ds);
        if (rc) return rc;
        *lds_bytes_max = std::max(*lds_bytes_max, (int)plan.lds_bytes);
        *tiles_total += plan.ntx * plan.nty;
        ngroups++;
        l0 += nl;
    }
    size_t o = 0;
    for (int l = 1; l < nlevels; l++)
        for (int y = 0; y < lh[l]; y++) {
            memcpy(out + o, &lv[l][(size_t)y * pitch[l]], lw[l]);
            o += lw[l];
        }
    return ngroups;
}

int vslamh_cells(int level, int lw, int lh, uint16_t* out5, int cap) {
    std::vector<vslam::HostCell> c;
    vslam::build_cells(level, lw, lh, c);
    for (int i = 0; i < (int)c.size() && i < cap; i++) {
        out5[5 * i] = c[i].level; out5[5 * i + 1] = c[i].x0; out5[5 * i + 2] = c[i].y0;
        out5[5 * i + 3] = c[i].x1; out5[5 * i + 4] = c[i].y1;
    }
    return (int)c.size();
}

int vslamh_bands(int level, int lw, int lh, int max_cells, int max_width, uint32_t* out8, int cap) {
    std::vector<vslam::HostCell> c;
    vslam::build_cells(level, lw, lh, c);
    std::vector<vslam::HostBand> b;
    vslam::build_bands(c, max_cells, max_width, b);
    for (int i = 0; i < (int)b.size() && i < cap; i++) {
        uint32_t* o = out8 + 8 * i;
        o[0] = b[i].cell0; o[1] = b[i].level; o[2] = b[i].ncell; o[3] = b[i].wcell;
        o[4] = b[i].x0; o[5] = b[i].y0; o[6] = b[i].ww; o[7] = b[i].wh;
    }
    return (int)b.size();
}

int vslamh_octree(const int32_t* xyr, int n, int W, int H, int N, int32_t* out_xyr, int cap) {
    std::vector<vslam::Cand> c(n), o;
    for (int i = 0; i < n; i++) {
        c[i].x = (int16_t)xyr[3 * i]; c[i].y = (int16_t)xyr[3 * i + 1]; c[i].response = (uint8_t)xyr[3 * i + 2];
    }
    if (!vslam::distribute_octree(c.data(), n, W, H, N, o)) return -1;
    for (int i = 0; i < (int)o.size() && i < cap; i++) {
        out_xyr[3 * i] = o[i].x; out_xyr[3 * i + 1] = o[i].y; out_xyr[3 * i + 2] = o[i].response;
    }
    return (int)o.size();
}

int vslamh_grid_query(const vslam_kp* kps, int n, int W, int H, float x, float y, float r, int minL, int maxL,
                      int* out, int cap) {
    vslam::FrameGrid g;
    g.build(kps, n, W, H);
    std::vector<int> v;
    g.query(x, y, r, minL, maxL, v);
    for (int i = 0; i < (int)v.size() && i < cap; i++) out[i] = v[i];
    return (int)v.size();
}

int vslamh_search_init(const vslam_kp* kps1, int n1, const vslam_kp* kps2, int n2, const uint8_t* dmat_full,
                       int W, int H, float* prevMatched, int32_t* matches12, int window, float nnratio,
                       int checkOri) {
    std::vector<int> rows(n1), cols(n2);
    for (int i = 0; i < n1; i++) rows[i] = i;
    for (int i = 0; i < n2; i++) cols[i] = i;
    const float b[4] = {0.0f, (float)W, 0.0f, (float)H};
    return vslam::search_for_initialization_replay(kps1, n1, kps2, n2, dmat_full, rows.data(), cols.data(), n2,
                                                   b, prevMatched, matches12, window, nnratio, checkOri != 0);
}

int vslamh_search_init_bounds(const vslam_kp* kps1, int n1, const vslam_kp* kps2, int n2, const uint8_t* dmat_full,
                              const float* bounds, float* prevMatched, int32_t* matches12, int window, float nnratio,
                              int checkOri) {
    std::vector<int> rows(n1), cols(n2);
    for (int i = 0; i < n1; i++) rows[i] = i;
    for (int i = 0; i < n2; i++) cols[i] = i;
    return vslam::search_for_initialization_replay(kps1, n1, kps2, n2, dmat_full, rows.data(), cols.data(), n2,
                                                   bounds, prevMatched, matches12, window, nnratio, checkOri != 0);
}

int vslamh_undistort_points(const float* cam, const float* dist, int ndist, const float* xy, int n, float* out) {
    if (ndist != 4 && ndist != 5) return -1;
    float d[5] = {0, 0, 0, 0, 0};
    for (int i = 0; i < ndist; i++) d[i] = dist[i];
    for (int i = 0; i < n; i++) vslam_ud::frame_undistort(xy[2 * i], xy[2 * i + 1], cam, d, &out[2 * i], &out[2 * i + 1]);
    return 0;
}

int vslamh_image_bounds(const float* cam, const float* dist, int ndist, int cols, int rows, float* b) {
    if (ndist != 4 && ndist != 5) return -1;
    float d[5] = {0, 0, 0, 0, 0};
    for (int i = 0; i < ndist; i++) d[i] = dist[i];
    vslam_ud::image_bounds(cam, d, cols, rows, b);
    return 0;
}
// ... 108 lines not shown
```

vi_slam_amd/csrc/vslam_host.h:

```cpp
#ifndef VSLAM_HOST_H
#define VSLAM_HOST_H

#include <cstdint>
#include <functional>
#include <vector>

#include "../../include/vslam_fe.h"

#define VSLAM_FAST_BORDER 16

namespace vslam {

struct ExtractorTables {
    int nlevels = 0;
    std::vector<float> scale, inv_scale, sigma2, inv_sigma2;
    std::vector<int> quota;
    int umax[16];
    std::vector<int8_t> disc_u, disc_v;
};
void build_tables(int nfeatures, float scaleFactor, int nlevels, ExtractorTables& t);

void level_size(const ExtractorTables& t, int w, int h, int level, int* lw, int* lh);

struct ResizeTables {
    std::vector<uint16_t> xtab, ytab;
    std::vector<int16_t> xa, yb;
};
void build_resize_tables(int sw, int sh, int dw, int dh, ResizeTables& r);
bool build_resize_quads(const ResizeTables& r, int sw, int dw, std::vector<uint16_t>& qbase,
                        std::vector<uint32_t>& quads);

struct PyrTileLevel {
    int16_t c0, nc;
    int16_t r0, nr;
    int16_t sq0, sq1;
    int16_t sr0, sr1;
    uint32_t lds_off;
    uint32_t pitch;
    uint32_t rt_off;
};
struct PyrGroupPlan {
    int l0 = 0, nl = 0;
    int ntx = 0, nty = 0;
    size_t lds_bytes = 0;
    std::vector<PyrTileLevel> tiles;
};
struct PyrLevelTables {
    int sw, sh, dw, dh;
    ResizeTables r;
    std::vector<uint16_t> qbase;
    std::vector<uint32_t> quads;
};
bool build_pyramid_group(const std::vector<const PyrLevelTables*>& tabs, int l0, size_t max_lds, PyrGroupPlan& plan,
                         int rows_override = -1 );
int emulate_pyramid_group(const PyrGroupPlan& plan, const std::vector<const PyrLevelTables*>& tabs,
                          const uint8_t* src, int sstride, int readable_w, std::vector<uint8_t*>& dst,
                          const std::vector<int>& dstride);

struct HostCell {
    uint16_t level, x0, y0, x1, y1;
};
void build_cells(int level, int lw, int lh, std::vector<HostCell>& out);

struct HostBand {
    uint32_t cell0;
    uint16_t level, ncell, wcell;
    uint16_t x0, y0, ww, wh;
};
void build_bands(const std::vector<HostCell>& cells, int max_cells, int max_width, std::vector<HostBand>& out);

struct BandWords {
    uint32_t cell0;
    uint32_t lnw;
    uint32_t xy;
    uint32_t wh;
};
struct BandTables {
    std::vector<BandWords> bands;
    std::vector<uint8_t> classes;
    int max_wh = 0, max_iw = 0, max_cells = 0;
    bool ok = false;
};
void pack_bands(const std::vector<HostBand>& hb, int nlevels, BandTables& out);

int keypoint_capacity(const int* quota, const int* lw, const int* lh, int nlevels, int nfeatures);

struct OctPlan {
    int32_t N[VSLAM_MAX_LEVELS], H[VSLAM_MAX_LEVELS], nIni[VSLAM_MAX_LEVELS], selOff[VSLAM_MAX_LEVELS];
    int32_t fineD[VSLAM_MAX_LEVELS], lutOff[VSLAM_MAX_LEVELS], lutW[VSLAM_MAX_LEVELS];
    float hX[VSLAM_MAX_LEVELS];
    int32_t selStride = 0, maxNodes = 0, fineLdsOff = 0, fineLdsBytes = 0;
    std::vector<uint32_t> lut;
    bool fits = false;
};
void plan_octree(const int* quota, const int* lw, const int* lh, const int* cell_first, int nlevels, int forced_depth,
                 size_t budget, const std::function<size_t(int)>& node_bytes, OctPlan& P);

struct Cand {
    int16_t x, y;
    uint8_t response;
};

bool distribute_octree(const Cand* cands, int n, int W, int H, int N, std::vector<Cand>& out);

void build_oct_lut(int W, int H, int D, std::vector<uint32_t>& xs, std::vector<uint32_t>& ys);
uint32_t oct_key_path(int x, int y, int W, int H, int depth);

void compute_three_maxima(const int* histo_sizes, int L, int& ind1, int& ind2, int& ind3);

struct FrameGrid {
    static const int COLS = 64, ROWS = 48;
    float minX, maxX, minY, maxY, invW, invH;
    std::vector<int> cell_start;
    std::vector<int> cell_items;
    const vslam_kp* kps;
    int n;
    void build(const vslam_kp* k, int n_, int imgW, int imgH);
    void build(const vslam_kp* k, int n_, const float bounds[4]);
    void query(float x, float y, float r, int minLevel, int maxLevel, std::vector<int>& out) const;
};

int search_for_initialization_replay(const vslam_kp* kps1, int n1, const vslam_kp* kps2, int n2,
                                     const uint8_t* dmat, const int* row_of_i1, const int* col_of_i2,
                                     int ncols, const float bounds[4], float* prevMatched, int32_t* matches12,
                                     int windowSize, float nnratio, bool checkOri);

}
#endif
```

vi_slam_amd/csrc/vslam_image_kernels.hip:

```cpp
#include "vslam_kernels.h"
#include "vslam_wave.h"

__device__ __forceinline__ const uint8_t* level_base_v2(const uint8_t* pyr, size_t slot_stride,
                                                        const BatchSrc& src, const LevelGeom& lg, int level,
                                                        int slot, int* pitch) {
    if (level == 0) {
        *pitch = (int)src.pitch0[slot];
        return src.l0[slot];
    }
    *pitch = lg.pitch;
    return pyr + (size_t)slot * slot_stride + lg.off;
}

__device__ __forceinline__ int refl101_v2(int p, int len) {
    if (p < 0) p = -p;
    if (p >= len) p = 2 * (len - 1) - p;
    return min(max(p, 0), len - 1);
}

#define BV_OUTW 248

__device__ __forceinline__ uint32_t udot4(uint32_t a, uint32_t b, uint32_t c) {
    return __builtin_amdgcn_udot4(a, b, c, false);
}

struct BlurTapsV2 {
    uint32_t l0, c0, l1, c1, r1, l2, c2, r2, c3, r3;
    uint32_t k[7];
};

#ifndef BLUR_WPB
#define BLUR_WPB 4
#endif
typedef unsigned short ushort2b __attribute__((ext_vector_type(2)));
__device__ __forceinline__ uint32_t udot2_u16(uint32_t a, uint32_t b, uint32_t c) {
    return __builtin_amdgcn_udot2(__builtin_bit_cast(ushort2b, a), __builtin_bit_cast(ushort2b, b), c, false);
}
__global__ void __launch_bounds__(64 * BLUR_WPB)
k_blur7_v2(const uint8_t* __restrict__ pyr, size_t slot_stride, BatchSrc src, PyramidGeom g, uint8_t* blur,
           const uint32_t* __restrict__ tasks, int ntasks, int nslots, int rows_per_task, BlurTapsV2 T) {
    const int lane = threadIdx.x & 63;
    const int tpb = (ntasks + BLUR_WPB - 1) / BLUR_WPB, nwork = tpb * nslots, per_xcd = (nwork + 7) >> 3;
    const int wk = (int)(blockIdx.x & 7) * per_xcd + (int)(blockIdx.x >> 3);
    if (wk >= nwork) return;
    const int slot = wk / tpb;
    const int task = (wk - slot * tpb) * BLUR_WPB + (threadIdx.x >> 6);
    if (task >= ntasks) return;
    const uint32_t td = (uint32_t)__builtin_amdgcn_readfirstlane((int)tasks[task]);
    const int level = td >> 24, rc = (td >> 12) & 0xFFF, strip = td & 0xFFF;
    const LevelGeom lg = g.lv[level];
    int pitch;
    const uint8_t* img = level_base_v2(pyr, slot_stride, src, lg, level, slot, &pitch);
    uint8_t* out = blur + (size_t)slot * slot_stride + lg.off;
    const int w = lg.w, h = lg.h;
    const int ox0 = min(strip * BV_OUTW, max(w - BV_OUTW, 0));
    const int x = ox0 - 4 + lane * 4;
    const int y0 = rc * rows_per_task;
    const int nrows = min(rows_per_task, h - y0);
    int bx[4];
#pragma unroll
    for (int k = 0; k < 4; k++) bx[k] = refl101_v2(x + k, w);
    const int bc = min(min(min(bx[0], bx[1]), min(bx[2], bx[3])), w - 8);
    const uint32_t sel = (uint32_t)(bx[0] - bc) | ((uint32_t)(bx[1] - bc) << 8) | ((uint32_t)(bx[2] - bc) << 16) |
                         ((uint32_t)(bx[3] - bc) << 24);

    auto load_row = [&](int yy) -> uint2 {
        const uint32_t* row = (const uint32_t*)(img + ((uint32_t)refl101_v2(yy, h) * (uint32_t)pitch + (uint32_t)bc));
        return make_uint2(row[0], row[1]);
    };
    auto hpass = [&](uint2 raw, uint32_t* o) {
        const uint32_t Cw = __builtin_amdgcn_perm(raw.y, raw.x, sel);
        const uint32_t Lw = (uint32_t)__builtin_amdgcn_update_dpp((int)Cw, (int)Cw, 0x138, 0xf, 0xf, false);
        const uint32_t Rw = (uint32_t)__builtin_amdgcn_update_dpp((int)Cw, (int)Cw, 0x130, 0xf, 0xf, false);
        o[0] = udot4(Lw, T.l0, udot4(Cw, T.c0, 0));
        o[1] = udot4(Lw, T.l1, udot4(Cw, T.c1, udot4(Rw, T.r1, 0)));
        o[2] = udot4(Lw, T.l2, udot4(Cw, T.c2, udot4(Rw, T.r2, 0)));
        o[3] = udot4(Cw, T.c3, udot4(Rw, T.r3, 0));
    };
    const uint32_t W01 = T.k[0] | (T.k[1] << 16), W23 = T.k[2] | (T.k[3] << 16), W45 = T.k[4] | (T.k[5] << 16);
    uint32_t pr[6][4];
    uint32_t prev[4];
    {
        uint32_t o[4];
        hpass(load_row(y0 - 3), prev);
#pragma unroll
        for (int r = 1; r < 6; r++) {
            hpass(load_row(y0 - 3 + r), o);
#pragma unroll
            for (int c = 0; c < 4; c++) {
                pr[r - 1][c] = prev[c] | (o[c] << 16);
                prev[c] = o[c];
            }
        }
    }
    const bool writer = lane >= 1 && lane <= 62 && x < w;
    uint2 nw[6];
#pragma unroll
    for (int u = 0; u < 6; u++) nw[u] = load_row(y0 + 3 + u);
    for (int rb = 0; rb < nrows; rb += 6) {
#pragma unroll
        for (int u = 0; u < 6; u++) {
            const int r = rb + u;
            if (r < nrows) {
                uint32_t o[4];
                hpass(nw[u], o);
                if (r + 6 < nrows) nw[u] = load_row(y0 + r + 9);
                uint32_t px[4];
#pragma unroll
                for (int c = 0; c < 4; c++) {
                    uint32_t acc = __umul24(T.k[6], o[c]) + 32768u;
                    acc = udot2_u16(pr[(u + 4) % 6][c], W45, acc);
                    acc = udot2_u16(pr[(u + 2) % 6][c], W23, acc);
                    acc = udot2_u16(pr[u][c], W01, acc);
                    px[c] = min(acc >> 16, 255u);
                    pr[(u + 5) % 6][c] = prev[c] | (o[c] << 16);
                    prev[c] = o[c];
                }
                if (writer) {
                    uint8_t* op = out + ((uint32_t)(y0 + r) * (uint32_t)lg.pitch + (uint32_t)x);
                    if (x + 3 < w) *(uint32_t*)op = px[0] | (px[1] << 8) | (px[2] << 16) | (px[3] << 24);
                    else {
                        op[0] = (uint8_t)px[0];
                        if (x + 1 < w) op[1] = (uint8_t)px[1];
                        if (x + 2 < w) op[2] = (uint8_t)px[2];
                    }
                }
            }
        }
    }
}

void vk_blur7_v2(hipStream_t st, const uint8_t* pyr, size_t slot_stride, const BatchSrc& src, const PyramidGeom& g,
                 uint8_t* blur, const uint32_t* tasks, int ntasks, const int32_t taps[7], int rows_per_task,
                 int nslots) {
    BlurTapsV2 T;
    const uint32_t k0 = taps[0], k1 = taps[1], k2 = taps[2], k3 = taps[3], k4 = taps[4], k5 = taps[5], k6 = taps[6];
    auto pk = [](uint32_t b0, uint32_t b1, uint32_t b2, uint32_t b3) { return b0 | (b1 << 8) | (b2 << 16) | (b3 << 24); };
    T.l0 = pk(0, k0, k1, k2); T.c0 = pk(k3, k4, k5, k6);
    T.l1 = pk(0, 0, k0, k1);  T.c1 = pk(k2, k3, k4, k5); T.r1 = pk(k6, 0, 0, 0);
    T.l2 = pk(0, 0, 0, k0);   T.c2 = pk(k1, k2, k3, k4); T.r2 = pk(k5, k6, 0, 0);
    T.c3 = pk(k0, k1, k2, k3); T.r3 = pk(k4, k5, k6, 0);
    for (int i = 0; i < 7; i++) T.k[i] = taps[i];
    const int nwork = ((ntasks + BLUR_WPB - 1) / BLUR_WPB) * nslots;
    hipLaunchKernelGGL(k_blur7_v2, dim3(((nwork + 7) / 8) * 8), dim3(64 * BLUR_WPB), 0, st, pyr, slot_stride, src, g, blur, tasks, ntasks,
                       nslots, rows_per_task, T);
}


__device__ __forceinline__ int imin3v(int a, int b, int c) {
    int r;
    asm("v_min3_i32 %0, %1, %2, %3" : "=v"(r) : "v"(a), "v"(b), "v"(c));
    return r;
}
__device__ __forceinline__ int imax3v(int a, int b, int c) {
    int r;
    asm("v_max3_i32 %0, %1, %2, %3" : "=v"(r) : "v"(a), "v"(b), "v"(c));
    return r;
}

template <int SIGN, int P>
__device__ __forceinline__ int fast_half_score(const uint8_t* c) {
    const int v = c[0];
    int d[16];
#define RD(k, off) d[k] = SIGN > 0 ? v - (int)c[off] : (int)c[off] - v
    RD(0, 3 * P);   RD(1, 3 * P + 1);   RD(2, 2 * P + 2);    RD(3, P + 3);
    RD(4, 3);        RD(5, -P + 3);      RD(6, -2 * P + 2);   RD(7, -3 * P + 1);
    RD(8, -3 * P);  RD(9, -3 * P - 1);  RD(10, -2 * P - 2);  RD(11, -P - 3);
    RD(12, -3);      RD(13, P - 3);      RD(14, 2 * P - 2);   RD(15, 3 * P - 1);
#undef RD
    int lo3[16];
#pragma unroll
    for (int k = 0; k < 16; k++) lo3[k] = imin3v(d[k], d[(k + 1) & 15], d[(k + 2) & 15]);
    int A = -256;
#pragma unroll
    for (int k = 0; k < 16; k += 2)
        A = imax3v(A, imin3v(lo3[k], lo3[(k + 3) & 15], lo3[(k + 6) & 15]),
                   imin3v(lo3[k + 1], lo3[(k + 4) & 15], lo3[(k + 7) & 15]));
    return A;
}

__device__ __forceinline__ uint32_t pk_sub_sat16(uint32_t a, uint32_t b) {
    uint32_t r;
    asm("v_pk_sub_u16 %0, %1, %2 clamp" : "=v"(r) : "v"(a), "v"(b));
    return r;
}
__device__ __forceinline__ uint32_t pk_min16(uint32_t a, uint32_t b) {
    uint32_t r;
    asm("v_pk_min_u16 %0, %1, %2" : "=v"(r) : "v"(a), "v"(b));
    return r;
}
__device__ __forceinline__ uint32_t pk_max16(uint32_t a, uint32_t b) {
    uint32_t r;
    asm("v_pk_max_u16 %0, %1, %2" : "=v"(r) : "v"(a), "v"(b));
    return r;
}
template <int SIGN, int P>
__device__ __forceinline__ uint32_t fast_pair_score(const uint8_t* ca, const uint8_t* cb) {
#define RING(off) (SIGN > 0 ? pk_sub_sat16(v, (uint32_t)ca[off] | ((uint32_t)cb[off] << 16)) \
                            : pk_sub_sat16((uint32_t)ca[off] | ((uint32_t)cb[off] << 16), v))
    const uint32_t v = (uint32_t)ca[0] | ((uint32_t)cb[0] << 16);
    uint32_t S1[8], P1[8], S2[8], P2[8];
    S1[0] = RING(3);           S1[1] = RING(-P + 3);      S1[2] = RING(-2 * P + 2);  S1[3] = RING(-3 * P + 1);
    S1[4] = RING(-3 * P);      S1[5] = RING(-3 * P - 1);  S1[6] = RING(-2 * P - 2);  S1[7] = RING(-P - 3);
    P1[0] = S1[0];
#pragma unroll
    for (int i = 1; i < 7; i++) P1[i] = pk_min16(P1[i - 1], S1[i]);
#pragma unroll
    for (int i = 6; i >= 0; i--) S1[i] = pk_min16(S1[i], S1[i + 1]);
    P1[7] = S1[0];
    __builtin_amdgcn_sched_barrier(0);
    S2[0] = RING(-3);          S2[1] = RING(P - 3);       S2[2] = RING(2 * P - 2);   S2[3] = RING(3 * P - 1);
    S2[4] = RING(3 * P);       S2[5] = RING(3 * P + 1);   S2[6] = RING(2 * P + 2);   S2[7] = RING(P + 3);
#undef RING
    P2[0] = S2[0];
#pragma unroll
    for (int i = 1; i < 7; i++) P2[i] = pk_min16(P2[i - 1], S2[i]);
#pragma unroll
    for (int i = 6; i >= 0; i--) S2[i] = pk_min16(S2[i], S2[i + 1]);
    P2[7] = S2[0];
    uint32_t best = pk_min16(S1[0], P2[0]);
#pragma unroll
    for (int i = 1; i < 8; i++) best = pk_max16(best, pk_min16(S1[i], P2[i]));
#pragma unroll
    for (int i = 0; i < 8; i++) best = pk_max16(best, pk_min16(S2[i], P1[i]));
    return best;
// ... 9 lines not shown
    asm("v_dot2_i32_i16 %0, %4, %8, 0\n\t"
        "v_dot2_i32_i16 %1, %5, %9, 0\n\t"
        "v_dot2_i32_i16 %2, %6, %10, 0\n\t"
        "v_dot2_i32_i16 %3, %7, %11, 0\n\t"
        "s_nop 3"
        : "=&v"(r0), "=&v"(r1), "=&v"(r2), "=&v"(r3)
        : "v"(t0), "v"(t1), "v"(t2), "v"(t3), "v"(cf.x), "v"(cf.y), "v"(cf.z), "v"(cf.w));
    *h0 = r0; *h1 = r1; *h2 = r2; *h3 = r3;
}

__global__ void __launch_bounds__(256)
k_resize_level_v2(uint8_t* pyr, size_t slot_stride, BatchSrc src, LevelGeom sg, LevelGeom dg, int src_level,
                  const uint16_t* __restrict__ qbase, const ResizeQuad* __restrict__ quads,
                  const uint16_t* __restrict__ ytab, const int16_t* __restrict__ yb, int nq) {
    const int q = blockIdx.x * 64 + (threadIdx.x & 63);
    const int dy = blockIdx.y * 4 + (threadIdx.x >> 6);
    const int slot = blockIdx.z;
    if (q >= nq || dy >= dg.h) return;
    int spitch;
    const uint8_t* S = level_base_v2(pyr, slot_stride, src, sg, src_level, slot, &spitch);
    const int sy0 = ytab[2 * dy], sy1 = ytab[2 * dy + 1];
    const int b0 = yb[2 * dy], b1 = yb[2 * dy + 1];
    const int base = qbase[q];
    const uint4 sel = *(const uint4*)quads[q].sel;
    const uint4 cf = *(const uint4*)quads[q].coef;
    const uint32_t* r0 = (const uint32_t*)(S + (size_t)sy0 * spitch + base);
    const uint32_t* r1 = (const uint32_t*)(S + (size_t)sy1 * spitch + base);
    const uint32_t lo0 = r0[0], hi0 = r0[1], lo1 = r1[0], hi1 = r1[1];
    uint32_t out = 0;
#define RZ_ONE(j, SEL, CF)                                                                                 \
    {                                                                                                      \
        const int h0 = hdot2(__builtin_amdgcn_perm(hi0, lo0, SEL), CF);                                    \
        const int h1 = hdot2(__builtin_amdgcn_perm(hi1, lo1, SEL), CF);                                    \
        const int v = (((__mul24(b0, h0 >> 4)) >> 16) + ((__mul24(b1, h1 >> 4)) >> 16) + 2) >> 2;         \
        out |= (uint32_t)(v & 0xFF) << (8 * (j));                                                          \
    }
    RZ_ONE(0, sel.x, cf.x)
    RZ_ONE(1, sel.y, cf.y)
    RZ_ONE(2, sel.z, cf.z)
    RZ_ONE(3, sel.w, cf.w)
#undef RZ_ONE
    *(uint32_t*)(pyr + (size_t)slot * slot_stride + dg.off + (size_t)dy * dg.pitch + 4 * q) = out;
}

void vk_resize_level_v2(hipStream_t st, uint8_t* pyr, size_t slot_stride, const BatchSrc& src, const LevelGeom& sg,
                        const LevelGeom& dg, int src_level, const uint16_t* qbase, const ResizeQuad* quads,
                        const uint16_t* ytab, const int16_t* yb, int nslots) {
    const int nq = (dg.w + 3) / 4;
    dim3 grid((nq + 63) / 64, (dg.h + 3) / 4, nslots);
    hipLaunchKernelGGL(k_resize_level_v2, grid, dim3(256), 0, st, pyr, slot_stride, src, sg, dg, src_level, qbase,
                       quads, ytab, yb, nq);
}

__device__ __forceinline__ uint4 pyr_load16_tail(const uint8_t* p, int nvalid) {
    uint32_t t[4] = {0, 0, 0, 0};
    const int nd = nvalid >> 2, nbyte = nvalid & 3;
#pragma unroll
    for (int i = 0; i < 4; i++) {
        if (i < nd) t[i] = *(const uint32_t*)(p + 4 * i);
        else if (i == nd) {
            if (nbyte > 0) t[i] |= (uint32_t)p[4 * i];
            if (nbyte > 1) t[i] |= (uint32_t)p[4 * i + 1] << 8;
            if (nbyte > 2) t[i] |= (uint32_t)p[4 * i + 2] << 16;
        }
    }
    return make_uint4(t[0], t[1], t[2], t[3]);
}

struct PyrTileU {
    int c0, nc, r0, nr, sq0, sq1, sr0, sr1;
    uint32_t lds_off, pitch, rt_off;
};
__device__ __forceinline__ PyrTileU pyr_tile_uniform(const PyrTileDev& t) {
    PyrTileU u;
#define PTU(f) u.f = __builtin_amdgcn_readfirstlane((int)t.f)
    PTU(c0); PTU(nc); PTU(r0); PTU(nr); PTU(sq0); PTU(sq1); PTU(sr0); PTU(sr1);
#undef PTU
    u.lds_off = (uint32_t)__builtin_amdgcn_readfirstlane((int)t.lds_off);
    u.pitch = (uint32_t)__builtin_amdgcn_readfirstlane((int)t.pitch);
    u.rt_off = (uint32_t)__builtin_amdgcn_readfirstlane((int)t.rt_off);
    return u;
}

template <int NT>
__global__ void __launch_bounds__(NT)
k_pyramid_group(uint8_t* pyr, size_t slot_stride, BatchSrc src, PyrGroupDev G, int nslots, uint8_t* reset_cand,
                size_t cand_stride, int32_t* reset_err) {
    extern __shared__ __align__(16) uint8_t psm[];
    constexpr int NW = NT / 64;
    const int lane = threadIdx.x & 63;
    const int wave = __builtin_amdgcn_readfirstlane((int)(threadIdx.x >> 6));
    if (reset_cand && blockIdx.x == 0) {
        if ((int)threadIdx.x < nslots) *(uint2*)(reset_cand + (size_t)threadIdx.x * cand_stride) = make_uint2(0u, 0u);
        if (reset_err && threadIdx.x < 4) reset_err[threadIdx.x] = 0;
    }
    const int nwork = G.ntiles * nslots, per_xcd = (nwork + 7) >> 3;
    const int wk = (int)(blockIdx.x & 7) * per_xcd + (int)(blockIdx.x >> 3);
    if (wk >= nwork) return;
    const int slot = wk / G.ntiles, tile = wk - slot * G.ntiles;
    const PyrTileDev* T = G.tiles + (size_t)tile * (G.nl + 1);
    const PyrTileDev S0 = T[0];
    if (S0.nr <= 0 || S0.nc <= 0) return;

    uint4 qsel[VSLAM_PYR_GROUP_LEVELS], qcf[VSLAM_PYR_GROUP_LEVELS];
    int qloc[VSLAM_PYR_GROUP_LEVELS];
#pragma unroll
    for (int j = 1; j <= VSLAM_PYR_GROUP_LEVELS; j++) {
        qsel[j - 1] = qcf[j - 1] = make_uint4(0, 0, 0, 0);
        qloc[j - 1] = 0;
        if (j <= G.nl) {
            const PyrTileDev D = T[j];
            if (lane < (D.nc >> 2)) {
                const int q = (D.c0 >> 2) + lane;
                qloc[j - 1] = (int)G.qbase[j - 1][q] - T[j - 1].c0;
                qsel[j - 1] = *(const uint4*)G.quads[j - 1][q].sel;
                qcf[j - 1] = *(const uint4*)G.quads[j - 1][q].coef;
            }
            uint2* rt = (uint2*)(psm + D.rt_off);
            for (int i = threadIdx.x; i < D.nr; i += NT) {
                const int r = D.r0 + i;
                rt[i] = make_uint2(*(const uint32_t*)(G.ytab[j - 1] + 2 * r), *(const uint32_t*)(G.yb[j - 1] + 2 * r));
            }
        }
    }
    {
        int spitch;
        const uint8_t* img = level_base_v2(pyr, slot_stride, src, G.lg[0], G.l0, slot, &spitch);
        const int readable = G.l0 == 0 ? G.readable_w0 : spitch;
        const int last_row = G.lg[0].h - 1;
        const uint32_t s0pitch = (uint32_t)__builtin_amdgcn_readfirstlane((int)S0.pitch);
        const int nch = (int)s0pitch >> 4, rpi = 64 / nch;
        const int rsub = lane / nch, ch = lane - rsub * nch;
        const bool lact = rsub < rpi;
        const int col = S0.c0 + 16 * ch;
        for (int kb = 0; kb * NW * rpi < S0.nr; kb += 4) {
            uint4 v[4];
#pragma unroll
            for (int u = 0; u < 4; u++) {
                const int row = ((kb + u) * NW + wave) * rpi + rsub;
                v[u] = make_uint4(0, 0, 0, 0);
                if (lact && row < S0.nr) {
                    const uint8_t* gp = img + mad24u_s((uint32_t)(S0.r0 + row), (uint32_t)spitch, (uint32_t)col);
                    if (col + 16 <= readable || (G.l0 == 0 && S0.r0 + row < last_row)) v[u] = *(const uint4*)gp;
                    else if (col < readable) v[u] = pyr_load16_tail(gp, readable - col);
                }
            }
#pragma unroll
            for (int u = 0; u < 4; u++) {
                const int row = ((kb + u) * NW + wave) * rpi + rsub;
                if (lact && row < S0.nr) *(uint4*)(psm + mad24u_s((uint32_t)row, s0pitch, S0.lds_off + 16u * (uint32_t)ch)) = v[u];
            }
        }
    }
    __syncthreads();
#pragma unroll
    for (int j = 1; j <= VSLAM_PYR_GROUP_LEVELS; j++) {
        if (j > G.nl) break;
        const PyrTileU S = pyr_tile_uniform(T[j - 1]), D = pyr_tile_uniform(T[j]);
        if (lane < (D.nc >> 2) && D.nr > 0) {
            const int q = (D.c0 >> 2) + lane;
            const int loc = qloc[j - 1];
            const uint32_t sh = (uint32_t)(loc & 3);
            const uint4 sel = qsel[j - 1], cf = qcf[j - 1];
            const int sp = (int)S.pitch, dp = (int)D.pitch;
            const int sbase = (int)S.lds_off + (loc & ~3) - __mul24((int)S.r0, sp);
            const int dbase = (int)D.lds_off + 4 * lane - __mul24((int)D.r0, dp);
            const bool qstore = q >= D.sq0 && q < D.sq1;
            uint8_t* gout = pyr + (size_t)slot * slot_stride + G.lg[j].off + 4 * (size_t)q;
            const int gpitch = G.lg[j].pitch;
            const uint2* rt = (const uint2*)(psm + D.rt_off) - D.r0;
            const int band = (D.nr + NW - 1) / NW;
            const int rb = D.r0 + wave * band, re = min(rb + band, D.r0 + D.nr);
            int prev_sy = -1;
            int hp0 = 0, hp1 = 0, hp2 = 0, hp3 = 0;
#define PYR_HPASS(SY, H0, H1, H2, H3)                                                                        \
    {                                                                                                         \
        const uint32_t* pr_ = (const uint32_t*)(psm + sbase + __mul24((int)(SY), sp));                        \
        const uint32_t x0_ = pr_[0], x1_ = pr_[1], x2_ = pr_[2];                                             \
        const uint32_t lo_ = __builtin_amdgcn_alignbyte(x1_, x0_, sh), hi_ = __builtin_amdgcn_alignbyte(x2_, x1_, sh); \
        hdot2x4(__builtin_amdgcn_perm(hi_, lo_, sel.x), __builtin_amdgcn_perm(hi_, lo_, sel.y),                \
                __builtin_amdgcn_perm(hi_, lo_, sel.z), __builtin_amdgcn_perm(hi_, lo_, sel.w), cf, &H0, &H1, &H2, &H3); \
        H0 >>= 4; H1 >>= 4; H2 >>= 4; H3 >>= 4;                                                               \
    }
            for (int r = rb; r < re; r++) {
                const uint2 e = rt[r];
                const int sy0 = __builtin_amdgcn_readfirstlane((int)(e.x & 0xFFFF));
                const int sy1 = __builtin_amdgcn_readfirstlane((int)(e.x >> 16));
                const int b0 = (int)(int16_t)(e.y & 0xFFFF), b1 = (int)e.y >> 16;
                int g0, g1, g2, g3;
                if (sy0 == prev_sy) {
                    g0 = hp0; g1 = hp1; g2 = hp2; g3 = hp3;
                } else
                    PYR_HPASS(sy0, g0, g1, g2, g3)
                if (sy1 != sy0) PYR_HPASS(sy1, hp0, hp1, hp2, hp3)
                else {
                    hp0 = g0; hp1 = g1; hp2 = g2; hp3 = g3;
                }
                prev_sy = sy1;
                const uint32_t v0 = (uint32_t)(((__mul24(b0, g0) >> 16) + (__mul24(b1, hp0) >> 16) + 2) >> 2);
                const uint32_t v1 = (uint32_t)(((__mul24(b0, g1) >> 16) + (__mul24(b1, hp1) >> 16) + 2) >> 2);
                const uint32_t v2 = (uint32_t)(((__mul24(b0, g2) >> 16) + (__mul24(b1, hp2) >> 16) + 2) >> 2);
                const uint32_t v3 = (uint32_t)(((__mul24(b0, g3) >> 16) + (__mul24(b1, hp3) >> 16) + 2) >> 2);
                const uint32_t out = (v0 & 0xFF) | ((v1 & 0xFF) << 8) | ((v2 & 0xFF) << 16) | (v3 << 24);
                *(uint32_t*)(psm + dbase + __mul24(r, dp)) = out;
                if (qstore && r >= D.sr0 && r < D.sr1) *(uint32_t*)(gout + (size_t)r * gpitch) = out;
            }
#undef PYR_HPASS
        }
        __syncthreads();
    }
}

void vk_pyramid_group(hipStream_t st, uint8_t* pyr, size_t slot_stride, const BatchSrc& src, const PyrGroupDev& G,
                      size_t lds_bytes, int nslots, uint8_t* reset_cand, size_t cand_stride, int32_t* reset_err) {
    const int nwork = G.ntiles * nslots;
    hipLaunchKernelGGL(k_pyramid_group<256>, dim3(((nwork + 7) / 8) * 8), dim3(256), lds_bytes, st, pyr, slot_stride, src, G, nslots,
                       reset_cand, cand_stride, reset_err);
}

typedef unsigned short ushort2v __attribute__((ext_vector_type(2)));
__device__ __forceinline__ uint32_t pk_sub_sat(uint32_t a, uint32_t b) {
    uint32_t r;
    asm("v_pk_sub_u16 %0, %1, %2 clamp" : "=v"(r) : "v"(a), "v"(b));
    return r;
}
__device__ __forceinline__ uint32_t pk_add(uint32_t a, uint32_t b) {
    uint32_t r;
    asm("v_pk_add_u16 %0, %1, %2" : "=v"(r) : "v"(a), "v"(b));
    return r;
}
__device__ __forceinline__ uint32_t pk_min(uint32_t a, uint32_t b) {
    uint32_t r;
    asm("v_pk_min_u16 %0, %1, %2" : "=v"(r) : "v"(a), "v"(b));
    return r;
}
__device__ __forceinline__ uint32_t pk_max(uint32_t a, uint32_t b) {
    uint32_t r;
    asm("v_pk_max_u16 %0, %1, %2" : "=v"(r) : "v"(a), "v"(b));
    return r;
}
template <int CTRL, int ROW_MASK>
__device__ __forceinline__ uint32_t dpp_or0(uint32_t v) {
    return (uint32_t)__builtin_amdgcn_update_dpp(0, (int)v, CTRL, ROW_MASK, 0xf, false);
}
__device__ __forceinline__ uint32_t wave_incl_scan(uint32_t v) {
    v += dpp_or0<0x111, 0xf>(v);
    v += dpp_or0<0x112, 0xf>(v);
    v += dpp_or0<0x114, 0xf>(v);
    v += dpp_or0<0x118, 0xf>(v);
    v += dpp_or0<0x142, 0xa>(v);
    v += dpp_or0<0x143, 0xc>(v);
    return v;
}

__device__ __forceinline__ uint32_t lds_addr(const void* p) { return (uint32_t)(uintptr_t)p; }
__device__ __forceinline__ uint64_t half_lo_nonzero(uint32_t x) {
    uint64_t m;
    asm("v_cmp_ne_u32_sdwa %0, %1, %2 src0_sel:WORD_0 src1_sel:DWORD" : "=s"(m) : "v"(x), "v"(0u));
    return m;
}
__device__ __forceinline__ uint64_t half_hi_nonzero(uint32_t x) {
    uint64_t m;
    asm("v_cmp_lt_u32_e64 %0, %1, %2" : "=s"(m) : "s"(0xFFFFu), "v"(x));
    return m;
}
__device__ __forceinline__ uint32_t lane_select(uint64_t m, uint32_t a, uint32_t b) {
    uint32_t r;
    asm("v_cndmask_b32_e64 %0, %1, %2, %3" : "=v"(r) : "v"(b), "v"(a), "s"(m));
    return r;
}
__device__ __forceinline__ uint32_t lane_rank(uint64_t m) {
    return __builtin_amdgcn_mbcnt_hi((uint32_t)(m >> 32), __builtin_amdgcn_mbcnt_lo((uint32_t)m, 0u));
}
__device__ __forceinline__ void lds_store_b16_masked2(uint64_t m, uint64_t mX, uint32_t at, uint32_t code, uint32_t codeX) {
    uint64_t save;
    asm volatile("s_mov_b64 %0, exec\n\t"
                 "s_mov_b64 exec, %1\n\tds_write_b16 %3, %4\n\t"
                 "s_cmp_eq_u64 %2, 0\n\ts_cbranch_scc1 1f\n\t"
                 "s_mov_b64 exec, %2\n\tds_write_b16 %3, %5\n"
                 "1:\n\ts_mov_b64 exec, %0"
                 : "=&s"(save) : "s"(m), "s"(mX), "v"(at), "v"(code), "v"(codeX) : "memory", "scc");
}
__device__ __forceinline__ uint32_t lds_add_rtn(uint32_t addr, uint32_t v) {
    uint32_t r;
    asm volatile("ds_add_rtn_u32 %0, %1, %2\n\ts_waitcnt lgkmcnt(0)" : "=v"(r) : "v"(addr), "v"(v) : "memory");
    return r;
}

#ifdef VSLAM_FAST_WGREC
#define FAST_WG_RECORDS 65536
__device__ unsigned long long g_fast_wg[FAST_WG_RECORDS * 4];
extern "C" int vslam_dbg_fast_wg_records(unsigned long long* out, int n) {
    if (n > FAST_WG_RECORDS) n = FAST_WG_RECORDS;
    if (hipMemcpyFromSymbol(out, HIP_SYMBOL(g_fast_wg), sizeof(unsigned long long) * 4 * (size_t)n) != hipSuccess) return -3;
    return n;
}
#endif
#ifdef VSLAM_FAST_STAMPS
__device__ unsigned long long g_fast_stamps[16];
#define FSTAMP(k) do { if (tid == 0) { const unsigned long long t_ = __builtin_amdgcn_s_memtime(); atomicAdd(&g_fast_stamps[k], t_ - fst_); fst_ = t_; } } while (0)
// ... 715 lines not shown
```

vi_slam_amd/csrc/vslam_kernels.h:

```cpp
#ifndef VSLAM_KERNELS_H
#define VSLAM_KERNELS_H

#include "vslam_tuning.h"
#include "vslam_device.h"

void vk_upload_disc(const int umax[16]);

void vk_resize_level(hipStream_t st, uint8_t* pyr, size_t slot_stride, const BatchSrc& src,
                     const LevelGeom& sg, const LevelGeom& dg, int src_level, const uint16_t* xtab,
                     const int16_t* xa, const uint16_t* ytab, const int16_t* yb, int nslots);

void vk_hamming_matrix(hipStream_t st, const uint8_t* q, int nq, const uint8_t* t, int nt, uint8_t* out);
int vk_hamming_top2_batch_split(int nprob, int max_nq, int max_nt);
void vk_hamming_top2_batch(hipStream_t st, const Top2Jobs& jobs, int nprob, int max_nq, int nrows, int nsplit, uint32_t* part,
                           int32_t* idx2, int32_t* dist2);

void vk_blur7_v2(hipStream_t st, const uint8_t* pyr, size_t slot_stride, const BatchSrc& src, const PyramidGeom& g,
                 uint8_t* blur, const uint32_t* tasks, int ntasks, const int32_t taps[7], int rows_per_task,
                 int nslots);
void vk_pyramid_group(hipStream_t st, uint8_t* pyr, size_t slot_stride, const BatchSrc& src, const PyrGroupDev& G,
                      size_t lds_bytes, int nslots, uint8_t* reset_cand = nullptr, size_t cand_stride = 0,
                      int32_t* reset_err = nullptr);
void vk_fast_cells_v3(hipStream_t st, const uint8_t* pyr, size_t slot_stride, const BatchSrc& src,
                      const PyramidGeom& g, const CellDesc* cells, int ncells, uint8_t* cand_region,
                      size_t cand_stride, int iniTh, int minTh, int tile_rows, int max_window_w, int max_px, int nslots);
int vk_fast_bands_check(int max_wh, int max_iw, int max_cells_per_band);
void vk_fast_bands(hipStream_t st, const uint8_t* pyr, size_t slot_stride, const BatchSrc& src, const PyramidGeom& g,
                   const BandDesc* bands, int nbands, const uint8_t* classes, const CellDesc* cells, int ncells, uint8_t* cand_region,
                   size_t cand_stride, int iniTh, int minTh, int max_wh, int max_iw, int nslots);
void vk_resize_level_v2(hipStream_t st, uint8_t* pyr, size_t slot_stride, const BatchSrc& src, const LevelGeom& sg,
                        const LevelGeom& dg, int src_level, const uint16_t* qbase, const ResizeQuad* quads,
                        const uint16_t* ytab, const int16_t* yb, int nslots);
size_t vk_octree_lds_bytes(int maxNodes);
int vk_octree_set_max_lds(size_t bytes);
void vk_octree(hipStream_t st, const uint8_t* cand_region, size_t cand_stride, int ncells, const OctParams& P,
               uint32_t* keys_a, uint32_t* aux_a, void* sorted_a, size_t pts_stride,
               uint32_t* sel_xyr, int32_t* sel_cnt, int32_t* err_flag, int nlevels, int nslots, int32_t* deep_flags,
               int regkeys, int threads = 1024);
void vk_assign_out(hipStream_t st, const OctParams& P, const PyramidGeom& g, uint32_t* sel_xyr, int32_t* sel_cnt, int lap0,
                   int lap1, SelKp* sel, int32_t* slot_counts, int cap, int32_t* err_flag, int nslots,
                   const int32_t* deep_flags);
void vk_orient_describe_dev(hipStream_t st, const uint8_t* pyr, const uint8_t* blur, size_t slot_stride,
                            const BatchSrc& src, const PyramidGeom& g, const SelKp* sel,
                            const int32_t* slot_counts, const int8_t* pattern, vslam_kp* kps, uint8_t* desc,
                            int cap, int atan_fma, int nslots, int kpw_override = -1);

void vk_dbg_sincos(hipStream_t st, const float* x, int n, float* s, float* c);
void vk_dbg_logf(hipStream_t st, const float* x, int n, float* y);
void vk_dbg_atan2(hipStream_t st, const float* y, const float* x, int n, int fma, float* a);

void vk_stereo(hipStream_t st, const StereoJobs& jobs, int njobs, int maxNL, int maxNR, const PyramidGeom& g,
               const uint8_t* pyrL, size_t strideL, const BatchSrc& srcL, const uint8_t* pyrR, size_t strideR,
               const BatchSrc& srcR, float mbf, float maxD, uint32_t* best, float* uRight, float* depth,
               int32_t* sad, int cap, int max_band, uint8_t* rows_scratch);
size_t vk_stereo_rows_bytes(int njobs, int nrows, int max_band, int cap);
void vk_hamming_matrix_batch(hipStream_t st, const MatJobs& jobs, int njobs, int maxr, int maxc, const int32_t* idx,
                             uint8_t* tmp, uint8_t* out);
size_t vk_search_init_lds(int cap, int max_c2);
size_t vk_search_init_scratch_bytes(int npairs, int max_c2, int M);
int vk_search_init_set_max_lds(size_t bytes);
void vk_search_init(hipStream_t st, const InitJobs& jobs, int npairs, int cap, const SiBounds& bounds, int window,
                    float nnratio, int checkOri, int32_t* matches_out, float* prev_out, int32_t* nmatch_out,
                    int max_c2, int M, uint8_t* scratch, int* fallbacks, const vslam_tuning& T);
size_t vk_sbp_rank_lds(int nCur);
size_t vk_sbp_replay_lds(int nCur, int nLast);
size_t vk_sbp_scratch_bytes(int nLast, int M);
size_t vk_sbp_proj_bytes(int nLast);
int vk_sbp_set_max_lds(size_t bytes);
void vk_search_by_projection(hipStream_t st, const SbpJobs& JS, int njobs, int maxLast, int maxCur, int* fallbacks,
                             int forceSeq);
int vk_distinctive_set_max_lds(size_t bytes);
void vk_distinctive(hipStream_t st, const uint8_t* desc, const int32_t* offsets, int nsets, int maxN, int32_t* best);
void vk_unproject_stereo(hipStream_t st, const UnprojJobs& U, int njobs);
void vk_fuse_search(hipStream_t st, const FuseArgsDev& A);
void vk_reset_headers(hipStream_t st, uint8_t* d_cand, size_t cand_stride_bytes, int nimg, int32_t* d_err);
int vk_copy_ranges(hipStream_t st, const CopyRanges& R, const vslam_tuning& T = vslam_process_tuning());
void vk_undistort_kps(hipStream_t st, const vslam_kp* kps, const int32_t* counts, vslam_kp* ukps, int cap, int nimg,
                      const UdCam& cam);
void vk_undistort_xy(hipStream_t st, const float* xy, int n, float* out, const UdCam& cam);
void vk_pull_images(hipStream_t st, const BatchSrc& src, uint8_t* pyr, size_t slot_stride, uint32_t off0, int dpitch,
                    int w, int h, int nimg, int from_host, const vslam_tuning& T);
void vk_pack_slots(hipStream_t st, const vslam_kp* kps, const uint8_t* desc, const int32_t* counts, int cap, int first,
                   int nslots, uint8_t* dst, size_t slot_bytes);
void vk_gather_rows32(hipStream_t st, const uint8_t* src, const int32_t* idx, int n, uint8_t* dst);

#endif
```

vi_slam_amd/csrc/vslam_tuning.cpp:

```cpp
#include "vslam_tuning.h"

#include <cstddef>
#include <cstdlib>
#include <cstring>
#include <mutex>

namespace {
struct EnvField {
    const char* env;
    size_t off;
    const char* word1;
    const char* word2;
};
#define TF(name, field, w1, w2) {name, offsetof(vslam_tuning, field), w1, w2}
const EnvField kEnv[] = {
    TF("VSLAM_PYRAMID", pyramid_per_level, "levels", nullptr),
    TF("VSLAM_PYR_ROWS", pyr_rows, nullptr, nullptr),
    TF("VSLAM_BLUR_ROWS", blur_rows, nullptr, nullptr),
    TF("VSLAM_OCT_FINE_D", oct_fine_depth, nullptr, nullptr),
    TF("VSLAM_OCT_LDS_BUDGET_KB", oct_lds_budget_kb, nullptr, nullptr),
    TF("VSLAM_OCT_REGKEYS", oct_regkeys, nullptr, nullptr),
    TF("VSLAM_OCT_MAXITER", oct_max_iter, nullptr, nullptr),
    TF("VSLAM_OCT_DBG", oct_debug, nullptr, nullptr),
    TF("VSLAM_GRAPH", graphs, nullptr, nullptr),
    TF("VSLAM_H2D", h2d_route, "pull", "sdma"),
    TF("VSLAM_D2H", d2h_route, "kernel", "sdma"),
    TF("VSLAM_COPY_WGS", copy_wgs, nullptr, nullptr),
    TF("VSLAM_PULL_DEPTH", pull_depth, nullptr, nullptr),
    TF("VSLAM_INIT_TOPM", init_topm, nullptr, nullptr),
    TF("VSLAM_INIT_MATCH", init_match_host, "host", nullptr),
    TF("VSLAM_SBP_TOPM", sbp_topm, nullptr, nullptr),
    TF("VSLAM_SBP_MODE", sbp_sequential, "seq", nullptr),
    TF("VSLAM_SI_QPB", si_queries_per_block, nullptr, nullptr),
    TF("VSLAM_FG_NT", fg_threads, nullptr, nullptr),
    TF("VSLAM_WAIT", wait_spin, "spin", nullptr),
    TF("VSLAM_NUMA", numa, nullptr, nullptr),
    TF("VSLAM_HOST_PROF", host_prof, nullptr, nullptr),
    TF("VSLAM_STREAM_PRIORITY", stream_priority, nullptr, nullptr),
    TF("VSLAM_STAGE_SPLIT_EVENT", stage_split_event, nullptr, nullptr),
    TF("VSLAM_OCT_THREADS", oct_threads, nullptr, nullptr),
    TF("VSLAM_FAST_KERNEL", fast_kernel, nullptr, nullptr),
    TF("VSLAM_FAST_BAND_CELLS", fast_band_cells, nullptr, nullptr),
    TF("VSLAM_DESC_KPW", desc_kpw, nullptr, nullptr),
};
#undef TF
vslam_tuning g_process;
std::once_flag g_once;

int32_t& field(vslam_tuning& t, size_t off) { return *reinterpret_cast<int32_t*>(reinterpret_cast<char*>(&t) + off); }
}

extern "C" void vslam_tuning_init(vslam_tuning* t) {
    if (!t) return;
    int32_t* w = reinterpret_cast<int32_t*>(t);
    for (size_t i = 0; i < sizeof(vslam_tuning) / sizeof(int32_t); i++) w[i] = -1;
}

const vslam_tuning& vslam_process_tuning() {
    std::call_once(g_once, [] {
        vslam_tuning_init(&g_process);
        for (const EnvField& e : kEnv) {
            const char* v = getenv(e.env);
            if (!v || !*v) continue;
            int32_t x;
            if (e.word1 && !strcmp(v, e.word1)) x = 1;
            else if (e.word2 && !strcmp(v, e.word2)) x = 2;
            else if ((*v >= '0' && *v <= '9') || *v == '-') x = (int32_t)atoi(v);
            else continue;
            if (x >= 0) field(g_process, e.off) = x;
        }
    });
    return g_process;
}

void vslam_apply_tuning(vslam_tuning& t, const vslam_tuning* user) {
    if (!user) return;
    for (const EnvField& e : kEnv) {
        const int32_t u = *reinterpret_cast<const int32_t*>(reinterpret_cast<const char*>(user) + e.off);
        if (u >= 0) field(t, e.off) = u;
    }
}

vslam_tuning vslam_resolve_tuning(const vslam_tuning* user) {
    vslam_tuning t = vslam_process_tuning();
    vslam_apply_tuning(t, user);
    return t;
}
```

Before: 195,500 frames/s.

## Fuse the 7-tap Gaussian blur into the pyramid group kernel using LDS tiles

Computes the 7x7 Gaussian blur for selected pyramid levels inside the fused pyramid-group kernel, reading from the level tiles already resident in LDS. The separate blur kernel then skips those levels and is not launched at all when no levels remain. The tile planner widens each owned tile by a halo (1 quad horizontally, 3 rows vertically) so the blur inputs are present in LDS. The cost is more LDS per tile and extra work inside the pyramid kernel, which could cut occupancy or force a different tile split. The level loop is also changed from fully unrolled to a runtime loop, with a select over per-level registers.

```diff
diff --git a/include/vslam_fe.h b/include/vslam_fe.h
--- a/include/vslam_fe.h
+++ b/include/vslam_fe.h
@@ -68,6 +68,7 @@
     int32_t wave_prio;
     int32_t oct_precount;
     int32_t desc_kpw;
+    int32_t blur_separate;
     int32_t reserved[1];
 } vslam_tuning;
 void vslam_tuning_init(vslam_tuning* t);
@@ -381,6 +382,7 @@
 int vslam_dbg_logf(vslam_fe* fe, const float* x, int n, float* y);
 int vslam_fe_octree_stats(const vslam_fe* fe, unsigned long long* problems, unsigned long long* split_below_grid,
                           uint32_t* last_level_masks);
+int vslam_fe_blur_owners(const vslam_fe* fe, int32_t* owner);
 int vslam_fe_delivery_stats(const vslam_fe* fe, unsigned long long* transfers, unsigned long long* bytes);
 int vslam_dbg_octree_stamps(vslam_fe* fe, unsigned long long* out64);
 int vslam_dbg_search_init_fallbacks(vslam_fe* fe, int* count);
diff --git a/vi_slam_amd/__init__.py b/vi_slam_amd/__init__.py
--- a/vi_slam_amd/__init__.py
+++ b/vi_slam_amd/__init__.py
@@ -37,7 +37,7 @@
     "vslam_search_by_projection_sim3",
     "vslam_comm_unique_id", "vslam_comm_create", "vslam_comm_destroy", "vslam_comm_rank", "vslam_comm_world",
     "vslam_exchange_ring", "vslam_exchange_allgather", "vslam_host_alloc", "vslam_host_free",
-    "vslam_fe_stage_images_async", "vslam_fe_octree_stats", "vslam_fe_delivery_stats", "vslam_dbg_search_init_replay_stats", "vslam_tuning_init", "vslam_fe_set_tuning", "vslam_stereo_fisheye_candidates", "vslam_hamming_top2_batch", "vslam_hamming_top2_batch_dev_async", "vslam_fe_set_fast_gate",
+    "vslam_fe_stage_images_async", "vslam_fe_octree_stats", "vslam_fe_delivery_stats", "vslam_fe_blur_owners", "vslam_dbg_search_init_replay_stats", "vslam_tuning_init", "vslam_fe_set_tuning", "vslam_stereo_fisheye_candidates", "vslam_hamming_top2_batch", "vslam_hamming_top2_batch_dev_async", "vslam_fe_set_fast_gate",
     "vslam_voc_load", "vslam_voc_file_open", "vslam_voc_file_close", "vslam_voc_file_info", "vslam_voc_file_arrays",
     "vslam_voc_file_last_error", "vslam_dbg_qlz_decode",
     "vslam_fe_set_camera", "vslam_fe_slot_ukps", "vslam_fe_ukps_copy", "vslam_undistort_points", "vslam_fe_image_bounds",
@@ -90,7 +90,8 @@
                  "oct_debug", "graphs", "h2d_route", "d2h_route", "copy_wgs", "pull_depth",
                  "init_topm", "init_match_host", "sbp_topm", "sbp_sequential", "si_queries_per_block", "fg_threads",
                  "wait_spin", "numa", "host_prof", "stream_priority", "stage_split_event",
-                 "oct_threads", "fast_kernel", "fast_band_cells", "wave_prio", "oct_precount", "desc_kpw"]
+                 "oct_threads", "fast_kernel", "fast_band_cells", "wave_prio", "oct_precount", "desc_kpw",
+                 "blur_separate"]
 
 
 class _Tuning(C.Structure):
@@ -611,6 +612,12 @@
         _check(lib().vslam_fe_octree_stats(self._h, C.byref(a), C.byref(b), m))
         return a.value, b.value, [int(v) for v in m]
 
+    def blur_owners(self):
+        o = (C.c_int32 * self.nlevels)()
+        lib().vslam_fe_blur_owners.argtypes = [C.c_void_p, C.c_void_p]
+        _check(lib().vslam_fe_blur_owners(self._h, o))
+        return [int(v) for v in o]
+
     def delivery_stats(self):
         a, b = C.c_ulonglong(), C.c_ulonglong()
         lib().vslam_fe_delivery_stats.argtypes = [C.c_void_p, C.c_void_p, C.c_void_p]
diff --git a/vi_slam_amd/csrc/vslam_ctx.h b/vi_slam_amd/csrc/vslam_ctx.h
--- a/vi_slam_amd/csrc/vslam_ctx.h
+++ b/vi_slam_amd/csrc/vslam_ctx.h
@@ -63,8 +63,10 @@
         PyrGroupDev dev;
         size_t lds_bytes;
         PyrTileDev* d_tiles;
+        uint32_t blur_mask;
     };
     std::vector<PyrGroupCtx> pyr_groups;
+    int blur_owner[VSLAM_MAX_LEVELS];
     std::vector<vslam::HostCell> cells;
     int level_cell_first[VSLAM_MAX_LEVELS + 1] = {};
     CellDesc* d_cells = nullptr;
diff --git a/vi_slam_amd/csrc/vslam_fe.hip b/vi_slam_amd/csrc/vslam_fe.hip
--- a/vi_slam_amd/csrc/vslam_fe.hip
+++ b/vi_slam_amd/csrc/vslam_fe.hip
@@ -180,6 +180,7 @@
             quads.clear();
         }
     }
+    for (int l = 0; l < VSLAM_MAX_LEVELS; l++) fe->blur_owner[l] = -1;
     bool fused = fe->tune.pyramid_per_level != 1 && p.nlevels > 1;
     for (int l = 1; l < p.nlevels && fused; l++) fused = fe->d_quads[l] != nullptr;
     static_assert(sizeof(PyrTileDev) == sizeof(vslam::PyrTileLevel), "planner and kernel share the tile record");
@@ -193,11 +194,16 @@
         std::vector<const vslam::PyrLevelTables*> gt;
         for (int j = 1; j <= nl; j++) gt.push_back(&pyr_tabs[l0 + j]);
         vslam::PyrGroupPlan plan;
-        if (!vslam::build_pyramid_group(gt, l0, VSLAM_PYR_LDS_KB * 1024, plan, pyr_rows)) {
+        const uint32_t want = fe->tune.blur_separate == 0 ? vslam::pyr_group_blur_mask(l0, nl) : 0u;
+        if (!(want && vslam::build_pyramid_group(gt, l0, VSLAM_PYR_LDS_KB * 1024, plan, pyr_rows, want)) &&
+            !vslam::build_pyramid_group(gt, l0, VSLAM_PYR_LDS_KB * 1024, plan, pyr_rows)) {
             fused = false;
             break;
         }
         vslam_fe::PyrGroupCtx g;
+        g.blur_mask = plan.blur_mask;
+        for (int j = 0; j <= nl; j++)
+            if ((plan.blur_mask >> j) & 1) fe->blur_owner[l0 + j] = (int)fe->pyr_groups.size();
         memset(&g.dev, 0, sizeof(g.dev));
         g.dev.l0 = l0;
         g.dev.nl = nl;
@@ -220,6 +226,7 @@
     if (!fused) {
         for (auto& g : fe->pyr_groups) hipFree(g.d_tiles);
         fe->pyr_groups.clear();
+        for (int l = 0; l < VSLAM_MAX_LEVELS; l++) fe->blur_owner[l] = -1;
     }
     return VSLAM_OK;
 }
@@ -284,13 +291,14 @@
     else if (fe->B <= 2) fe->blur_rows = 8;
     std::vector<uint32_t> tasks;
     for (int l = 0; l < fe->p.nlevels; l++) {
+        if (fe->blur_owner[l] >= 0) continue;
         const int br = fe->blur_rows;
         const int ns = std::max(1, (fe->geom.lv[l].w + 247) / 248), nc = (fe->geom.lv[l].h + br - 1) / br;
         for (int c = 0; c < nc; c++)
             for (int s = 0; s < ns; s++) tasks.push_back(((uint32_t)l << 24) | ((uint32_t)c << 12) | (uint32_t)s);
     }
     fe->n_blur_tasks = (int)tasks.size();
-    UPLOAD(fe->d_blur_tasks, tasks.data(), tasks.size() * 4);
+    if (!tasks.empty()) UPLOAD(fe->d_blur_tasks, tasks.data(), tasks.size() * 4);
     return VSLAM_OK;
 }
 
@@ -465,6 +473,12 @@
     return VSLAM_OK;
 }
 
+extern "C" int vslam_fe_blur_owners(const vslam_fe* fe, int32_t* owner) {
+    if (!fe || !owner) return VSLAM_ERR_INVALID;
+    for (int l = 0; l < fe->p.nlevels; l++) owner[l] = fe->blur_owner[l];
+    return VSLAM_OK;
+}
+
 extern "C" int vslam_fe_delivery_stats(const vslam_fe* fe, unsigned long long* transfers, unsigned long long* bytes) {
     if (!fe) return VSLAM_ERR_INVALID;
     if (transfers) *transfers = fe->n_deliveries;
@@ -759,7 +773,8 @@
     bool first_group = true;
     for (const auto& g : fe->pyr_groups) {
         vk_pyramid_group(st, fe->d_pyr, fe->slot_stride, fe->src, g.dev, g.lds_bytes, nimg,
-                         first_group ? fe->d_cand : nullptr, fe->cand_stride, first_group ? d_errw : nullptr);
+                         first_group ? fe->d_cand : nullptr, fe->cand_stride, first_group ? d_errw : nullptr, fe->d_blur, g.blur_mask,
+                         fe->taps);
         first_group = false;
     }
     for (int l = 1; l < L && fe->pyr_groups.empty(); l++) {
@@ -806,8 +821,9 @@
 
 static int enqueue_blur(vslam_fe* fe, int nimg) {
     if (fe->profiling) HIPCHK(hipEventRecord(fe->ev_prof[3], fe->stream));
-    vk_blur7_v2(fe->stream, fe->d_pyr, fe->slot_stride, fe->src, fe->geom, fe->d_blur, fe->d_blur_tasks,
-                fe->n_blur_tasks, fe->taps, fe->blur_rows, nimg);
+    if (fe->n_blur_tasks > 0)
+        vk_blur7_v2(fe->stream, fe->d_pyr, fe->slot_stride, fe->src, fe->geom, fe->d_blur, fe->d_blur_tasks,
+                    fe->n_blur_tasks, fe->taps, fe->blur_rows, nimg);
     if (fe->profiling) HIPCHK(hipEventRecord(fe->ev_prof[4], fe->stream));
     return VSLAM_OK;
 }
diff --git a/vi_slam_amd/csrc/vslam_host.cpp b/vi_slam_amd/csrc/vslam_host.cpp
--- a/vi_slam_amd/csrc/vslam_host.cpp
+++ b/vi_slam_amd/csrc/vslam_host.cpp
@@ -138,8 +138,9 @@
 static inline int div_floor4(int x) { return x >> 2; }
 
 static bool plan_with(const std::vector<const PyrLevelTables*>& tabs, int l0, int ntx, int nty, size_t max_lds,
-                      PyrGroupPlan& plan) {
+                      uint32_t blur_mask, PyrGroupPlan& plan) {
     const int nl = (int)tabs.size();
+    plan.blur_mask = blur_mask;
     plan.l0 = l0;
     plan.nl = nl;
     plan.ntx = ntx;
@@ -153,16 +154,22 @@
             int nq0 = -1, nq1 = -1, nr0 = -1, nr1 = -1;
             for (int j = nl; j >= 0; j--) {
                 int oq0 = 0, oq1 = 0, or0 = 0, or1 = 0;
-                if (j >= 1) {
-                    const PyrLevelTables& t = *tabs[j - 1];
-                    const int nq = (t.dw + 3) / 4;
+                const bool blurred = (blur_mask >> j) & 1;
+                if (j >= 1 || blurred) {
+                    const int lw = j >= 1 ? tabs[j - 1]->dw : tabs[0]->sw, lh = j >= 1 ? tabs[j - 1]->dh : tabs[0]->sh;
+                    const int nq = (lw + 3) / 4;
                     oq0 = (int)((long long)tx * nq / ntx);
                     oq1 = (int)((long long)(tx + 1) * nq / ntx);
-                    or0 = (int)((long long)ty * t.dh / nty);
-                    or1 = (int)((long long)(ty + 1) * t.dh / nty);
+                    or0 = (int)((long long)ty * lh / nty);
+                    or1 = (int)((long long)(ty + 1) * lh / nty);
                     T[j].sq0 = (int16_t)oq0; T[j].sq1 = (int16_t)oq1; T[j].sr0 = (int16_t)or0; T[j].sr1 = (int16_t)or1;
+                    if (blurred && oq1 > oq0 && or1 > or0) {
+                        if (oq1 - oq0 > 64) return false;
+                        oq0 = std::max(oq0 - 1, 0); oq1 = std::min(oq1 + 1, nq);
+                        or0 = std::max(or0 - 3, 0); or1 = std::min(or1 + 3, lh);
+                    }
                 }
-                const bool own = j >= 1 && oq1 > oq0 && or1 > or0, need = nq1 > nq0 && nr1 > nr0;
+                const bool own = oq1 > oq0 && or1 > or0, need = nq1 > nq0 && nr1 > nr0;
                 if (!own && !need) { cq0[j] = cq1[j] = cr0[j] = cr1[j] = 0; }
                 else if (own && need) {
                     cq0[j] = std::min(oq0, nq0); cq1[j] = std::max(oq1, nq1);
@@ -203,7 +210,8 @@
     return lds_max <= max_lds;
 }
 
-bool build_pyramid_group(const std::vector<const PyrLevelTables*>& tabs, int l0, size_t max_lds, PyrGroupPlan& plan, int rows_override) {
+bool build_pyramid_group(const std::vector<const PyrLevelTables*>& tabs, int l0, size_t max_lds, PyrGroupPlan& plan, int rows_override,
+                         uint32_t blur_mask) {
     if (tabs.empty() || tabs.size() > VSLAM_MAX_LEVELS) return false;
     for (const PyrLevelTables* t : tabs)
         if (!t || t->qbase.empty()) return false;
@@ -215,14 +223,59 @@
 #define VSLAM_PYR_TILE_QUADS 52
 #endif
     for (int ntx = std::max(1, (nq1 + VSLAM_PYR_TILE_QUADS - 1) / VSLAM_PYR_TILE_QUADS); ntx <= std::max(1, nq1 / 8); ntx++)
-        if (plan_with(tabs, l0, ntx, nty, max_lds, plan)) return true;
+        if (plan_with(tabs, l0, ntx, nty, max_lds, blur_mask, plan)) return true;
     return false;
 }
 
 int emulate_pyramid_group(const PyrGroupPlan& plan, const std::vector<const PyrLevelTables*>& tabs,
                           const uint8_t* src, int sstride, int readable_w, std::vector<uint8_t*>& dst,
-                          const std::vector<int>& dstride) {
+                          const std::vector<int>& dstride, const int32_t* taps, const std::vector<uint8_t*>* bdst,
+                          const std::vector<int>* bstride, const std::vector<uint8_t*>* bcount) {
     const int nl = plan.nl;
+    auto blur_tile = [&](const PyrTileLevel& D, int j, const std::vector<uint8_t>& lds, const std::vector<uint8_t>& ok) -> int {
+        if (!taps || !bdst || !((plan.blur_mask >> j) & 1) || !(*bdst)[j] || D.sq1 <= D.sq0 || D.sr1 <= D.sr0) return 0;
+        const int w = j >= 1 ? tabs[j - 1]->dw : tabs[0]->sw, h = j >= 1 ? tabs[j - 1]->dh : tabs[0]->sh;
+        const int bs = (*bstride)[j];
+        for (int q = D.sq0; q < D.sq1; q++) {
+            const int x = 4 * q;
+            int xa[3];
+            uint32_t sel[3];
+            for (int g = 0; g < 3; g++) {
+                sel[g] = pyr_blur_window(x - 4 + 4 * g, x, w, &xa[g]);
+                if (xa[g] < D.c0 || xa[g] + 8 > D.c0 + (int)D.pitch) return -10;
+            }
+            for (int y = D.sr0; y < D.sr1; y++) {
+                int row[7][12];
+                for (int dy = 0; dy < 7; dy++) {
+                    int yy = y + dy - 3;
+                    if (yy < 0) yy = -yy;
+                    if (yy >= h) yy = 2 * (h - 1) - yy;
+                    yy = std::min(std::max(yy, 0), h - 1);
+                    if (yy < D.r0 || yy >= D.r0 + D.nr) return -11;
+                    for (int g = 0; g < 3; g++)
+                        for (int b = 0; b < 4; b++) {
+                            const int c = xa[g] + (int)((sel[g] >> (8 * b)) & 0xFF);
+                            const size_t a = D.lds_off + (size_t)(yy - D.r0) * D.pitch + (size_t)(c - D.c0);
+                            const bool used = 4 * g + b >= 1 && 4 * g + b <= 4 + std::min(3, w - 1 - x) + 3;
+                            if (used && (c < D.c0 || c >= D.c0 + D.nc || a >= lds.size())) return -12;
+                            if (used && !ok[a]) return -13;
+                            row[dy][4 * g + b] = a < lds.size() ? lds[a] : 0;
+                        }
+                }
+                for (int k = 0; k < 4 && x + k < w; k++) {
+                    uint32_t acc = 32768u;
+                    for (int dy = 0; dy < 7; dy++) {
+                        uint32_t hsum = 0;
+                        for (int dx = 0; dx < 7; dx++) hsum += (uint32_t)taps[dx] * (uint32_t)row[dy][4 + k - 3 + dx];
+                        acc += (uint32_t)taps[dy] * hsum;
+                    }
+                    (*bdst)[j][(size_t)y * bs + x + k] = (uint8_t)std::min(acc >> 16, 255u);
+                    if (bcount && (*bcount)[j]) (*bcount)[j][(size_t)y * bs + x + k]++;
+                }
+            }
+        }
+        return 0;
+    };
     std::vector<uint8_t> lds(plan.lds_bytes), ok(plan.lds_bytes);
     for (int tile = 0; tile < plan.ntx * plan.nty; tile++) {
         const PyrTileLevel* T = &plan.tiles[(size_t)tile * (nl + 1)];
@@ -239,6 +292,7 @@
                     ok[a] = 1;
                 }
             }
+        if (const int rc = blur_tile(T[0], 0, lds, ok)) return rc;
         for (int j = 1; j <= nl; j++) {
             const PyrLevelTables& t = *tabs[j - 1];
             const PyrTileLevel &S = T[j - 1], &D = T[j];
@@ -277,6 +331,7 @@
                             if (4 * q + k < dstride[j]) dst[j][(size_t)r * dstride[j] + 4 * q + k] = (uint8_t)(out >> (8 * k));
                 }
             }
+            if (const int rc = blur_tile(D, j, lds, ok)) return rc;
         }
     }
     return 0;
@@ -843,8 +898,9 @@
     return 0;
 }
 
-int vslamh_pyramid_fused(const uint8_t* img, int w, int h, size_t stride, int nfeatures, float scale, int nlevels,
-                         uint8_t* out, int* lds_bytes_max, int* tiles_total) {
+static int pyramid_fused_impl(const uint8_t* img, int w, int h, size_t stride, int nfeatures, float scale, int nlevels,
+                              uint8_t* out, int* lds_bytes_max, int* tiles_total, const int32_t* taps, int pyr_rows,
+                              uint8_t* out_blur, uint8_t* out_count) {
     vslam::ExtractorTables t;
     vslam::build_tables(nfeatures, scale, nlevels, t);
     std::vector<vslam::PyrLevelTables> tabs(nlevels);
@@ -862,6 +918,11 @@
         pitch[l] = (lw[l] + 127) & ~127;
         lv[l].assign((size_t)pitch[l] * lh[l], 0xEE);
     }
+    std::vector<std::vector<uint8_t>> bl(nlevels), bc(nlevels);
+    for (int l = 0; l < nlevels && taps; l++) {
+        bl[l].assign((size_t)pitch[l] * lh[l], 0xEE);
+        bc[l].assign((size_t)pitch[l] * lh[l], 0);
+    }
     for (int y = 0; y < h; y++) memcpy(&lv[0][(size_t)y * pitch[0]], img + (size_t)y * stride, w);
     int ngroups = 0;
     *lds_bytes_max = 0;
@@ -871,11 +932,13 @@
         std::vector<const vslam::PyrLevelTables*> gt;
         for (int j = 1; j <= nl; j++) gt.push_back(&tabs[l0 + j]);
         vslam::PyrGroupPlan plan;
-        if (!vslam::build_pyramid_group(gt, l0, 64 * 1024, plan)) return -101;
-        std::vector<uint8_t*> dst(nl + 1, nullptr);
-        std::vector<int> ds(nl + 1, 0);
+        if (!vslam::build_pyramid_group(gt, l0, 64 * 1024, plan, pyr_rows, taps ? vslam::pyr_group_blur_mask(l0, nl) : 0u)) return -101;
+        std::vector<uint8_t*> dst(nl + 1, nullptr), bd(nl + 1, nullptr), bn(nl + 1, nullptr);
+        std::vector<int> ds(nl + 1, 0), bs(nl + 1, 0);
         for (int j = 1; j <= nl; j++) { dst[j] = lv[l0 + j].data(); ds[j] = pitch[l0 + j]; }
-        const int rc = vslam::emulate_pyramid_group(plan, gt, lv[l0].data(), pitch[l0], l0 == 0 ? w : pitch[l0], dst, ds);
+        for (int j = 0; j <= nl && taps; j++) { bd[j] = bl[l0 + j].data(); bn[j] = bc[l0 + j].data(); bs[j] = pitch[l0 + j]; }
+        const int rc = vslam::emulate_pyramid_group(plan, gt, lv[l0].data(), pitch[l0], l0 == 0 ? w : pitch[l0], dst, ds, taps,
+                                                    &bd, &bs, &bn);
         if (rc) return rc;
         *lds_bytes_max = std::max(*lds_bytes_max, (int)plan.lds_bytes);
         *tiles_total += plan.ntx * plan.nty;
@@ -883,12 +946,32 @@
         l0 += nl;
     }
     size_t o = 0;
-    for (int l = 1; l < nlevels; l++)
+    for (int l = 1; l < nlevels && out; l++)
         for (int y = 0; y < lh[l]; y++) {
             memcpy(out + o, &lv[l][(size_t)y * pitch[l]], lw[l]);
             o += lw[l];
         }
+    o = 0;
+    for (int l = 0; l < nlevels && taps; l++)
+        for (int y = 0; y < lh[l]; y++) {
+            memcpy(out_blur + o, &bl[l][(size_t)y * pitch[l]], lw[l]);
+            memcpy(out_count + o, &bc[l][(size_t)y * pitch[l]], lw[l]);
+            o += lw[l];
+        }
     return ngroups;
+}
+
+int vslamh_pyramid_fused(const uint8_t* img, int w, int h, size_t stride, int nfeatures, float scale, int nlevels,
+                         uint8_t* out, int* lds_bytes_max, int* tiles_total) {
+    return pyramid_fused_impl(img, w, h, stride, nfeatures, scale, nlevels, out, lds_bytes_max, tiles_total, nullptr, -1, nullptr,
+                              nullptr);
+}
+
+int vslamh_pyramid_fused_blur(const uint8_t* img, int w, int h, size_t stride, int nfeatures, float scale, int nlevels,
+                              const int32_t* taps, int pyr_rows, uint8_t* out_blur, uint8_t* out_count, int* lds_bytes_max,
+                              int* tiles_total) {
+    return pyramid_fused_impl(img, w, h, stride, nfeatures, scale, nlevels, nullptr, lds_bytes_max, tiles_total, taps, pyr_rows,
+                              out_blur, out_count);
 }
 
 int vslamh_cells(int level, int lw, int lh, uint16_t* out5, int cap) {
diff --git a/vi_slam_amd/csrc/vslam_host.h b/vi_slam_amd/csrc/vslam_host.h
--- a/vi_slam_amd/csrc/vslam_host.h
+++ b/vi_slam_amd/csrc/vslam_host.h
@@ -43,6 +43,7 @@
     int l0 = 0, nl = 0;
     int ntx = 0, nty = 0;
     size_t lds_bytes = 0;
+    uint32_t blur_mask = 0;
     std::vector<PyrTileLevel> tiles;
 };
 struct PyrLevelTables {
@@ -52,10 +53,32 @@
     std::vector<uint32_t> quads;
 };
 bool build_pyramid_group(const std::vector<const PyrLevelTables*>& tabs, int l0, size_t max_lds, PyrGroupPlan& plan,
-                         int rows_override = -1 );
+                         int rows_override = -1 , uint32_t blur_mask = 0);
+inline uint32_t pyr_group_blur_mask(int l0, int nl) { return ((2u << nl) - 1u) & (l0 == 0 ? ~0u : ~1u); }
+#if defined(__HIPCC__)
+__host__ __device__
+#endif
+inline uint32_t pyr_blur_window(int p0, int x, int w, int* xa) {
+    const int pmin = x - 3, last = (x + 3 < w - 1 ? x + 3 : w - 1) + 3;
+    int col[4], lo = 1 << 30;
+    for (int b = 0; b < 4; b++) {
+        int p = p0 + b;
+        p = p < pmin ? pmin : p > last ? last : p;
+        if (p < 0) p = -p;
+        if (p >= w) p = 2 * (w - 1) - p;
+        p = p < 0 ? 0 : p > w - 1 ? w - 1 : p;
+        col[b] = p;
+        lo = p < lo ? p : lo;
+    }
+    *xa = lo & ~3;
+    return (uint32_t)(col[0] - *xa) | ((uint32_t)(col[1] - *xa) << 8) | ((uint32_t)(col[2] - *xa) << 16) |
+           ((uint32_t)(col[3] - *xa) << 24);
+}
 int emulate_pyramid_group(const PyrGroupPlan& plan, const std::vector<const PyrLevelTables*>& tabs,
                           const uint8_t* src, int sstride, int readable_w, std::vector<uint8_t*>& dst,
-                          const std::vector<int>& dstride);
+                          const std::vector<int>& dstride, const int32_t* taps = nullptr,
+                          const std::vector<uint8_t*>* bdst = nullptr, const std::vector<int>* bstride = nullptr,
+                          const std::vector<uint8_t*>* bcount = nullptr);
 
 struct HostCell {
     uint16_t level, x0, y0, x1, y1;
diff --git a/vi_slam_amd/csrc/vslam_image_kernels.hip b/vi_slam_amd/csrc/vslam_image_kernels.hip
--- a/vi_slam_amd/csrc/vslam_image_kernels.hip
+++ b/vi_slam_amd/csrc/vslam_image_kernels.hip
@@ -1,4 +1,5 @@
 #include "vslam_kernels.h"
+#include "vslam_host.h"
 #include "vslam_wave.h"
 
 __device__ __forceinline__ const uint8_t* level_base_v2(const uint8_t* pyr, size_t slot_stride,
@@ -36,6 +37,67 @@
 __device__ __forceinline__ uint32_t udot2_u16(uint32_t a, uint32_t b, uint32_t c) {
     return __builtin_amdgcn_udot2(__builtin_bit_cast(ushort2b, a), __builtin_bit_cast(ushort2b, b), c, false);
 }
+template <class Raw, class LoadRow, class HPass, class Store>
+__device__ __forceinline__ void blur7_march(int y0, int nrows, const BlurTapsV2& T, LoadRow load_row, HPass hpass, Store store) {
+    const uint32_t W01 = T.k[0] | (T.k[1] << 16), W23 = T.k[2] | (T.k[3] << 16), W45 = T.k[4] | (T.k[5] << 16);
+    uint32_t pr[6][4];
+    uint32_t prev[4];
+    {
+        uint32_t o[4];
+        hpass(load_row(y0 - 3), prev);
+#pragma unroll
+        for (int r = 1; r < 6; r++) {
+            hpass(load_row(y0 - 3 + r), o);
+#pragma unroll
+            for (int c = 0; c < 4; c++) {
+                pr[r - 1][c] = prev[c] | (o[c] << 16);
+                prev[c] = o[c];
+            }
+        }
+    }
+    Raw nw[6];
+#pragma unroll
+    for (int u = 0; u < 6; u++) nw[u] = load_row(y0 + 3 + u);
+    for (int rb = 0; rb < nrows; rb += 6) {
+#pragma unroll
+        for (int u = 0; u < 6; u++) {
+            const int r = rb + u;
+            if (r < nrows) {
+                uint32_t o[4];
+                hpass(nw[u], o);
+                if (r + 6 < nrows) nw[u] = load_row(y0 + r + 9);
+                uint32_t px[4];
+#pragma unroll
+                for (int c = 0; c < 4; c++) {
+                    uint32_t acc = __umul24(T.k[6], o[c]) + 32768u;
+                    acc = udot2_u16(pr[(u + 4) % 6][c], W45, acc);
+                    acc = udot2_u16(pr[(u + 2) % 6][c], W23, acc);
+                    acc = udot2_u16(pr[u][c], W01, acc);
+                    px[c] = min(acc >> 16, 255u);
+                    pr[(u + 5) % 6][c] = prev[c] | (o[c] << 16);
+                    prev[c] = o[c];
+                }
+                store(y0 + r, px);
+            }
+        }
+    }
+}
+
+__device__ __forceinline__ void blur7_hdots(uint32_t Lw, uint32_t Cw, uint32_t Rw, const BlurTapsV2& T, uint32_t* o) {
+    o[0] = udot4(Lw, T.l0, udot4(Cw, T.c0, 0));
+    o[1] = udot4(Lw, T.l1, udot4(Cw, T.c1, udot4(Rw, T.r1, 0)));
+    o[2] = udot4(Lw, T.l2, udot4(Cw, T.c2, udot4(Rw, T.r2, 0)));
+    o[3] = udot4(Cw, T.c3, udot4(Rw, T.r3, 0));
+}
+__device__ __forceinline__ void blur7_store4(uint8_t* op, int x, int w, const uint32_t* px) {
+    if (x + 3 < w) *(uint32_t*)op = px[0] | (px[1] << 8) | (px[2] << 16) | (px[3] << 24);
+    else {
+        op[0] = (uint8_t)px[0];
+        if (x + 1 < w) op[1] = (uint8_t)px[1];
+        if (x + 2 < w) op[2] = (uint8_t)px[2];
+    }
+}
+
 __global__ void __launch_bounds__(64 * BLUR_WPB)
 k_blur7_v2(const uint8_t* __restrict__ pyr, size_t slot_stride, BatchSrc src, PyramidGeom g, uint8_t* blur,
            const uint32_t* __restrict__ tasks, int ntasks, int nslots, int rows_per_task, BlurTapsV2 T) {
@@ -72,67 +134,15 @@
         const uint32_t Cw = __builtin_amdgcn_perm(raw.y, raw.x, sel);
         const uint32_t Lw = (uint32_t)__builtin_amdgcn_update_dpp((int)Cw, (int)Cw, 0x138, 0xf, 0xf, false);
         const uint32_t Rw = (uint32_t)__builtin_amdgcn_update_dpp((int)Cw, (int)Cw, 0x130, 0xf, 0xf, false);
-        o[0] = udot4(Lw, T.l0, udot4(Cw, T.c0, 0));
-        o[1] = udot4(Lw, T.l1, udot4(Cw, T.c1, udot4(Rw, T.r1, 0)));
-        o[2] = udot4(Lw, T.l2, udot4(Cw, T.c2, udot4(Rw, T.r2, 0)));
-        o[3] = udot4(Cw, T.c3, udot4(Rw, T.r3, 0));
+        blur7_hdots(Lw, Cw, Rw, T, o);
     };
-    const uint32_t W01 = T.k[0] | (T.k[1] << 16), W23 = T.k[2] | (T.k[3] << 16), W45 = T.k[4] | (T.k[5] << 16);
-    uint32_t pr[6][4];
-    uint32_t prev[4];
-    {
-        uint32_t o[4];
-        hpass(load_row(y0 - 3), prev);
-#pragma unroll
-        for (int r = 1; r < 6; r++) {
-            hpass(load_row(y0 - 3 + r), o);
-#pragma unroll
-            for (int c = 0; c < 4; c++) {
-                pr[r - 1][c] = prev[c] | (o[c] << 16);
-                prev[c] = o[c];
-            }
-        }
-    }
     const bool writer = lane >= 1 && lane <= 62 && x < w;
-    uint2 nw[6];
-#pragma unroll
-    for (int u = 0; u < 6; u++) nw[u] = load_row(y0 + 3 + u);
-    for (int rb = 0; rb < nrows; rb += 6) {
-#pragma unroll
-        for (int u = 0; u < 6; u++) {
-            const int r = rb + u;
-            if (r < nrows) {
-                uint32_t o[4];
-                hpass(nw[u], o);
-                if (r + 6 < nrows) nw[u] = load_row(y0 + r + 9);
-                uint32_t px[4];
-#pragma unroll
-                for (int c = 0; c < 4; c++) {
-                    uint32_t acc = __umul24(T.k[6], o[c]) + 32768u;
-                    acc = udot2_u16(pr[(u + 4) % 6][c], W45, acc);
-                    acc = udot2_u16(pr[(u + 2) % 6][c], W23, acc);
-                    acc = udot2_u16(pr[u][c], W01, acc);
-                    px[c] = min(acc >> 16, 255u);
-                    pr[(u + 5) % 6][c] = prev[c] | (o[c] << 16);
-                    prev[c] = o[c];
-                }
-                if (writer) {
-                    uint8_t* op = out + ((uint32_t)(y0 + r) * (uint32_t)lg.pitch + (uint32_t)x);
-                    if (x + 3 < w) *(uint32_t*)op = px[0] | (px[1] << 8) | (px[2] << 16) | (px[3] << 24);
-                    else {
-                        op[0] = (uint8_t)px[0];
-                        if (x + 1 < w) op[1] = (uint8_t)px[1];
-                        if (x + 2 < w) op[2] = (uint8_t)px[2];
-                    }
-                }
-            }
-        }
-    }
-}
-
-void vk_blur7_v2(hipStream_t st, const uint8_t* pyr, size_t slot_stride, const BatchSrc& src, const PyramidGeom& g,
-                 uint8_t* blur, const uint32_t* tasks, int ntasks, const int32_t taps[7], int rows_per_task,
-                 int nslots) {
+    blur7_march<uint2>(y0, nrows, T, load_row, hpass, [&](int y, const uint32_t* px) {
+        if (writer) blur7_store4(out + ((uint32_t)y * (uint32_t)lg.pitch + (uint32_t)x), x, w, px);
+    });
+}
+
+static BlurTapsV2 blur_taps_v2(const int32_t taps[7]) {
     BlurTapsV2 T;
     const uint32_t k0 = taps[0], k1 = taps[1], k2 = taps[2], k3 = taps[3], k4 = taps[4], k5 = taps[5], k6 = taps[6];
     auto pk = [](uint32_t b0, uint32_t b1, uint32_t b2, uint32_t b3) { return b0 | (b1 << 8) | (b2 << 16) | (b3 << 24); };
@@ -141,6 +151,13 @@
     T.l2 = pk(0, 0, 0, k0);   T.c2 = pk(k1, k2, k3, k4); T.r2 = pk(k5, k6, 0, 0);
     T.c3 = pk(k0, k1, k2, k3); T.r3 = pk(k4, k5, k6, 0);
     for (int i = 0; i < 7; i++) T.k[i] = taps[i];
+    return T;
+}
+
+void vk_blur7_v2(hipStream_t st, const uint8_t* pyr, size_t slot_stride, const BatchSrc& src, const PyramidGeom& g,
+                 uint8_t* blur, const uint32_t* tasks, int ntasks, const int32_t taps[7], int rows_per_task,
+                 int nslots) {
+    const BlurTapsV2 T = blur_taps_v2(taps);
     const int nwork = ((ntasks + BLUR_WPB - 1) / BLUR_WPB) * nslots;
     hipLaunchKernelGGL(k_blur7_v2, dim3(((nwork + 7) / 8) * 8), dim3(64 * BLUR_WPB), 0, st, pyr, slot_stride, src, g, blur, tasks, ntasks,
                        nslots, rows_per_task, T);
@@ -316,10 +333,50 @@
     return u;
 }
 
+struct PyrBlurRaw {
+    uint32_t l0, l1, c0, c1, r0, r1;
+};
+template <int NW>
+__device__ __forceinline__ void pyr_blur_tile(const uint8_t* psm, const PyrTileU& D, const LevelGeom& lg, uint8_t* out,
+                                              const BlurTapsV2& T, int lane, int wave) {
+    const int nsq = D.sq1 - D.sq0;
+    const int band = (D.sr1 - D.sr0 + NW - 1) / NW;
+    const int y0 = D.sr0 + wave * band, nrows = min(band, D.sr1 - y0);
+    if (nsq <= 0 || nrows <= 0) return;
+    const int w = lg.w, h = lg.h;
+    const int x = 4 * (D.sq0 + min(lane, nsq - 1));
+    uint32_t sel[3];
+    int off[3];
+#pragma unroll
+    for (int g = 0; g < 3; g++) {
+        int xa;
+        sel[g] = vslam::pyr_blur_window(x - 4 + 4 * g, x, w, &xa);
+        off[g] = (int)D.lds_off + (xa - D.c0) - __mul24(D.r0, (int)D.pitch);
+    }
+    const bool writer = lane < nsq;
+    uint8_t* op0 = out + (uint32_t)x;
+    blur7_march<PyrBlurRaw>(
+        y0, nrows, T,
+        [&](int yy) -> PyrBlurRaw {
+            const int rowoff = __mul24(refl101_v2(yy, h), (int)D.pitch);
+            const uint32_t* pl = (const uint32_t*)(psm + off[0] + rowoff);
+            const uint32_t* pc = (const uint32_t*)(psm + off[1] + rowoff);
+            const uint32_t* pr = (const uint32_t*)(psm + off[2] + rowoff);
+            return PyrBlurRaw{pl[0], pl[1], pc[0], pc[1], pr[0], pr[1]};
+        },
+        [&](const PyrBlurRaw& raw, uint32_t* o) {
+            blur7_hdots(__builtin_amdgcn_perm(raw.l1, raw.l0, sel[0]), __builtin_amdgcn_perm(raw.c1, raw.c0, sel[1]),
+                        __builtin_amdgcn_perm(raw.r1, raw.r0, sel[2]), T, o);
+        },
+        [&](int y, const uint32_t* px) {
+            if (writer) blur7_store4(op0 + (uint32_t)y * (uint32_t)lg.pitch, x, w, px);
+        });
+}
+
 template <int NT>
 __global__ void __launch_bounds__(NT)
 k_pyramid_group(uint8_t* pyr, size_t slot_stride, BatchSrc src, PyrGroupDev G, int nslots, uint8_t* reset_cand,
-                size_t cand_stride, int32_t* reset_err) {
+                size_t cand_stride, int32_t* reset_err, uint8_t* blur, uint32_t blur_mask, BlurTapsV2 BT) {
     extern __shared__ __align__(16) uint8_t psm[];
     constexpr int NW = NT / 64;
     const int lane = threadIdx.x & 63;
@@ -387,15 +444,24 @@
         }
     }
     __syncthreads();
-#pragma unroll
-    for (int j = 1; j <= VSLAM_PYR_GROUP_LEVELS; j++) {
+#pragma unroll 1
+    for (int j = 1; j <= G.nl + 1; j++) {
+        const PyrTileU S = pyr_tile_uniform(T[j - 1]);
+        const LevelGeom lgs = G.lg[j - 1];
+        if ((blur_mask >> (j - 1)) & 1)
+            pyr_blur_tile<NW>(psm, S, lgs, blur + (size_t)slot * slot_stride + lgs.off, BT, lane, wave);
         if (j > G.nl) break;
-        const PyrTileU S = pyr_tile_uniform(T[j - 1]), D = pyr_tile_uniform(T[j]);
+        const PyrTileU D = pyr_tile_uniform(T[j]);
         if (lane < (D.nc >> 2) && D.nr > 0) {
             const int q = (D.c0 >> 2) + lane;
-            const int loc = qloc[j - 1];
+            int loc = qloc[0];
+            uint4 sel = qsel[0], cf = qcf[0];
+#pragma unroll
+            for (int k = 1; k < VSLAM_PYR_GROUP_LEVELS; k++)
+                if (j == k + 1) {
+                    loc = qloc[k]; sel = qsel[k]; cf = qcf[k];
+                }
             const uint32_t sh = (uint32_t)(loc & 3);
-            const uint4 sel = qsel[j - 1], cf = qcf[j - 1];
             const int sp = (int)S.pitch, dp = (int)D.pitch;
             const int sbase = (int)S.lds_off + (loc & ~3) - __mul24((int)S.r0, sp);
             const int dbase = (int)D.lds_off + 4 * lane - __mul24((int)D.r0, dp);
@@ -446,10 +512,11 @@
 }
 
 void vk_pyramid_group(hipStream_t st, uint8_t* pyr, size_t slot_stride, const BatchSrc& src, const PyrGroupDev& G,
-                      size_t lds_bytes, int nslots, uint8_t* reset_cand, size_t cand_stride, int32_t* reset_err) {
+                      size_t lds_bytes, int nslots, uint8_t* reset_cand, size_t cand_stride, int32_t* reset_err, uint8_t* blur,
+                      uint32_t blur_mask, const int32_t taps[7]) {
     const int nwork = G.ntiles * nslots;
     hipLaunchKernelGGL(k_pyramid_group<256>, dim3(((nwork + 7) / 8) * 8), dim3(256), lds_bytes, st, pyr, slot_stride, src, G, nslots,
-                       reset_cand, cand_stride, reset_err);
+                       reset_cand, cand_stride, reset_err, blur, blur_mask, blur_taps_v2(taps));
 }
 
 typedef unsigned short ushort2v __attribute__((ext_vector_type(2)));
diff --git a/vi_slam_amd/csrc/vslam_kernels.h b/vi_slam_amd/csrc/vslam_kernels.h
--- a/vi_slam_amd/csrc/vslam_kernels.h
+++ b/vi_slam_amd/csrc/vslam_kernels.h
@@ -19,8 +19,8 @@
                  uint8_t* blur, const uint32_t* tasks, int ntasks, const int32_t taps[7], int rows_per_task,
                  int nslots);
 void vk_pyramid_group(hipStream_t st, uint8_t* pyr, size_t slot_stride, const BatchSrc& src, const PyrGroupDev& G,
-                      size_t lds_bytes, int nslots, uint8_t* reset_cand = nullptr, size_t cand_stride = 0,
-                      int32_t* reset_err = nullptr);
+                      size_t lds_bytes, int nslots, uint8_t* reset_cand, size_t cand_stride, int32_t* reset_err,
+                      uint8_t* blur, uint32_t blur_mask , const int32_t taps[7]);
 void vk_fast_cells_v3(hipStream_t st, const uint8_t* pyr, size_t slot_stride, const BatchSrc& src,
                       const PyramidGeom& g, const CellDesc* cells, int ncells, uint8_t* cand_region,
                       size_t cand_stride, int iniTh, int minTh, int tile_rows, int max_window_w, int max_px, int nslots);
diff --git a/vi_slam_amd/csrc/vslam_tuning.cpp b/vi_slam_amd/csrc/vslam_tuning.cpp
--- a/vi_slam_amd/csrc/vslam_tuning.cpp
+++ b/vi_slam_amd/csrc/vslam_tuning.cpp
@@ -42,6 +42,7 @@
     TF("VSLAM_FAST_KERNEL", fast_kernel, nullptr, nullptr),
     TF("VSLAM_FAST_BAND_CELLS", fast_band_cells, nullptr, nullptr),
     TF("VSLAM_DESC_KPW", desc_kpw, nullptr, nullptr),
+    TF("VSLAM_BLUR", blur_separate, "separate", nullptr),
 };
 #undef TF
 vslam_tuning g_process;
```

New measurement: 189,900 frames/s. 0.972x the previous value.
